# bdwsq1996/Effi-MVS-plus

Measured on NVIDIA B200. Metric: depth_maps_per_sec_1600x1184_5view, higher is better.
Workload: dtype hi+lo bf16 MMA x3, f32 accumulate (3-D regularization, fp32-grade) / f32 (warp, lookup, regression)

## Files before the change

### effi-mvs-plus_b200/capi.py

```python
from __future__ import annotations

import ctypes as C
import os

_HERE = os.path.dirname(os.path.abspath(__file__))
LIB_PATH = os.environ.get("EFFIMVS_LIB") or os.path.join(_HERE, "libeffimvs.so")

OK, EINVAL, EUNSUPPORTED, ECUDA, EWORKSPACE = 0, -1, -2, -3, -4
HYP_TENSOR, HYP_PLANES, HYP_LOCAL = 0, 1, 2
RANGE_SCALAR, RANGE_PIXEL = 0, 1
FEA_NCHW, FEA_NHWC = 0, 1
PREC_F32, PREC_BF16, PREC_BF16X3 = 0, 1, 2
WS_PREPARE, WS_RUN = 1, 2
CONV2D_BIAS, CONV2D_BIAS_RELU, CONV2D_ADD_RELU, CONV2D_GRU_GATES, CONV2D_GRU_UPDATE = 0, 1, 2, 3, 4
MAX_SRC_VIEWS = 16


class EffiMVSError(RuntimeError):
    def __init__(self, code, msg):
        super().__init__("libeffimvs error {}: {}".format(code, msg))
        self.code = code


if not os.path.exists(LIB_PATH):
    raise ImportError("libeffimvs.so is not built ({}); run __graft_entry__.build() -- the hot path has no "
                      "CPU or PyTorch fallback".format(LIB_PATH))

lib = C.CDLL(LIB_PATH)

_p, _i, _f, _sz = C.c_void_p, C.c_int, C.c_float, C.c_size_t
_pp = C.POINTER(C.c_void_p)

SIGNATURES = {
    "effimvs_last_error": (C.c_char_p, []),
    "effimvs_version": (_i, []),
    "effimvs_relative_projection_f32": (_i, [_p, _i, _i, _p, _p]),
    "effimvs_homo_warp_f32": (_i, [_p, _p, _p, _i, _i, _i, _i, _i, _i, _p, _p]),
    "effimvs_depth_range_samples_f32": (_i, [_p, _p, _i, _i, _i, _i, _p, _p]),
    "effimvs_depth_ranges_f32": (_i, [_p, _i, _i, _i, _p, _p, _p]),
    "effimvs_fusion_masks_f32": (_i, [_p, _p, _i, _i, _i, _i, _f, _f, _i, _i, _p, _p]),
    "effimvs_warp_corr_agg_f32": (_i, [_p, _pp, _i, _p, _p, _i, _p, _p, _i, _i, _i, _i, _i, _i, _i, _p, _p, _p]),
    "effimvs_warp_corr_views_f32": (_i, [_p, _pp, _i, _p, _p, _i, _i, _i, _i, _i, _i, _i, _p, _p, _p]),
    "effimvs_weighted_agg_f32": (_i, [_p, _p, _i, _i, _i, _i, _i, _p, _p]),
    "effimvs_volume_lookup_f32": (_i, [_p, _p, _p, _p, _i, _i, _i, _i, _i, _i, _i, _p, _p]),
    "effimvs_dynamic_cost_f32": (_i, [_p, _p, _p, _p, _p, _p, _i, _i, _i, _i, _i, _i, _p, _p]),
    "effimvs_softmax_regress_conf_f32": (_i, [_p, _p, _i, _i, _i, _i, _i, _p, _p, _p]),
    "effimvs_conv3d_f32": (_i, [_p, _p, _p, _p, _i, _i, _i, _i, _i, _i, _i, _i, _i, _i, _i, _p, _i, _i, _p]),
    "effimvs_conv3d_bf16_workspace_bytes": (_sz, [_i, _i, _i, _i, _i, _i, _i, _i, _i]),
    "effimvs_conv3d_bf16": (_i, [_p, _p, _p, _p, _i, _i, _i, _i, _i, _i, _i, _i, _i, _i, _p, _sz, _p, _p]),
    "effimvs_costreg_workspace_bytes": (_sz, [_i, _i, _i, _i, _i]),
    "effimvs_costreg_fpn3d": (_i, [_p, _pp, _pp, _i, _i, _i, _i, _i, _p, _sz, _p, _p]),
    "effimvs_cost_up_workspace_bytes": (_sz, [_i, _i, _i, _i, _i]),
    "effimvs_cost_up_small": (_i, [_p, _p, _pp, _pp, _i, _i, _i, _i, _i, _p, _sz, _p, _p]),
    "effimvs_costreg_fpn3d_ex": (_i, [_p, _pp, _pp, _i, _i, _i, _i, _i, _i, _p, _sz, _p, _p]),
    "effimvs_cost_up_small_ex": (_i, [_p, _p, _pp, _pp, _i, _i, _i, _i, _i, _i, _p, _sz, _p, _p]),
    "effimvs_gru_reset_f32": (_i, [_p, _p, _p, C.c_longlong, _i, _i, _p, _p]),
    "effimvs_gru_update_f32": (_i, [_p, _p, _p, _p, _p, C.c_longlong, _i, _i, _p, _p]),
    "effimvs_gru_delta_f32": (_i, [_p, _p, _p, _p, _p, _i, _i, _p, _p, _p]),
    "effimvs_inv_init_f32": (_i, [_p, _p, _p, _i, _i, _p, _p, _p]),
    "effimvs_delta_head_f32": (_i, [_p, _p, _p, _p, _p, _p, _i, _i, _i, _i, _p, _p, _p]),
    "effimvs_convex_upsample_f32": (_i, [_p, _p, _f, _p, _p, _p, _i, _i, _i, _i, _p, _p, _p]),
    "effimvs_convex_upsample_conv_f32": (_i, [_p, _i, _p, _p, _f, _p, _p, _p, _i, _i, _i, _i, _p, _p, _p]),
    "effimvs_encoder_head_f32": (_i, [_p, _p, _p, _p, _p, _p, _i, _i, _i, _i, _i, _p, _p]),
    "effimvs_encoder_head_hostw_f32": (_i, [_p, _p, _p, _i, _i, _i, _i, _i, _p, _p]),
    "effimvs_encoder_head_pack_host": (_i, [_p, _p, _p, _p, _i, _i, _p]),
    "effimvs_encoder_head_table_floats": (_i, [_i]),
    "effimvs_encoder_tail_f32": (_i, [_p, _p, _p, C.c_longlong, _i, _i, _p, _p]),
    "effimvs_encoder_tail_ctx_f32": (_i, [_p, _p, _p, _i, _i, _i, _p, _p, C.c_longlong, _i, _i, _p, _p]),
    "effimvs_conv2d_tf32_supported": (_i, [_i, _i]),
    "effimvs_conv2d_tf32_packed_bytes": (_sz, [_i, _i]),
    "effimvs_conv2d_tf32_pack": (_i, [_p, _i, _i, _p, _p]),
    "effimvs_conv2d_bf16x3_supported": (_i, [_i, _i]),
    "effimvs_conv2d_bf16x3_packed_bytes": (_sz, [_i, _i]),
    "effimvs_conv2d_bf16x3_pack": (_i, [_p, _i, _i, _p, _p]),
    "effimvs_conv2d_bf16x3": (_i, [_p, C.c_longlong, _i, _p, C.c_longlong, _i, _p, _p, _i, _i, _i, _i, _i,
                                   _p, C.c_longlong, _p, C.c_longlong, _p, C.c_longlong, _p]),
    "effimvs_conv2d_tf32": (_i, [_p, C.c_longlong, _i, _p, C.c_longlong, _i, _p, _p, _i, _i, _i, _i, _i,
                                 _p, C.c_longlong, _p, C.c_longlong, _p, C.c_longlong, _p]),
    "effimvs_gru_init_f32": (_i, [_p, C.c_longlong, _i, _i, _p, _p]),
    "effimvs_gru_init_ctx_f32": (_i, [_p, C.c_longlong, _i, _i, _p, _p, _p, _p, _p]),
    "effimvs_dtu_filter_f32": (_i, [_p, _p, _p, _p, C.POINTER(C.c_double), C.POINTER(C.c_float), _i, _i, _i, _f, _f, _i, _i, _i,
                                    _p, _p, _p, _p, _p, _p, _p]),
    "effimvs_images_u8_to_f32": (_i, [_p, C.c_longlong, _p, _p]),
    "effimvs_fusion_invert_cameras_f32": (_i, [_p, _p, _i, _i, _p, _p]),
    "effimvs_fusion_reproject_f32": (_i, [_p, _p, _p, _p, _p, _i, _i, _i, _i, _p, _p]),
    "effimvs_fusion_filter_f32": (_i, [_p, _p, _p, _p, _p, _p, _i, _i, _i, _i, _i, _i, _f, _f, _i, _f, _i, _p, _p, _p, _p, _p]),
}

for _name, (_res, _args) in SIGNATURES.items():
    _fn = getattr(lib, _name)
    _fn.restype = _res
    _fn.argtypes = _args


def last_error() -> str:
    return lib.effimvs_last_error().decode("utf-8", "replace")


def check(rc: int) -> None:
    if rc != OK:
        raise EffiMVSError(rc, last_error())


def ptr_array(ptrs):
    arr = (C.c_void_p * len(ptrs))(*[C.c_void_p(p) for p in ptrs])
    return C.cast(arr, _pp), arr
```

### effi-mvs-plus_b200/hotpath.py

```python
from __future__ import annotations

import collections
import functools
import os
import weakref

import torch

from . import capi, ops


def fold_bn(block, transposed: bool):
    bn = block.bn
    scale = bn.weight / torch.sqrt(bn.running_var + bn.eps)
    shift = bn.bias - bn.running_mean * scale
    w = block.conv.weight
    w = w * (scale.reshape(1, -1, 1, 1, 1) if transposed else scale.reshape(-1, 1, 1, 1, 1))
    return w.detach().float().contiguous(), shift.detach().float().contiguous()


class _FoldCache:

    def __init__(self):
        self._store = weakref.WeakKeyDictionary()

    def get(self, net, build):
        stamp = tuple((id(t), t._version, t.device) for t in list(net.parameters()) + list(net.buffers()))
        hit = self._store.get(net)
        if hit is None or hit[0] != stamp:
            hit = (stamp, build(net))
            self._store[net] = hit
        return hit[1]


def _inference_only(*tensors):
    if torch.is_grad_enabled() and any(torch.is_tensor(t) and t.requires_grad for t in tensors):
        raise RuntimeError("the CUDA hot path is inference only (no autograd formula): run it under torch.no_grad(), "
                           "or use upstream's PyTorch path for training / test-time adaptation")


class _WorkspaceCache:

    def __init__(self, cap: int = 24):
        self._store = collections.OrderedDict()
        self.cap = cap

    def get(self, key, nbytes, device):
        capturing = torch.cuda.is_current_stream_capturing() if torch.device(device).type == "cuda" else False
        ent = self._store.get(key)
        if ent is not None and ent["ws"].numel() < nbytes:
            if ent["pinned"]:
                raise RuntimeError("a regularization workspace captured in a CUDA graph is too small for this call")
            ent = None
        if ent is None:
            if capturing:
                raise RuntimeError("regularization workspace requested for the first time during CUDA-graph capture: "
                                   "run one eager forward of this shape before capturing")
            ent = {"ws": torch.empty(max(nbytes, 256), device=device, dtype=torch.uint8), "stamp": None, "pinned": False}
            self._store[key] = ent
            evictable = [k for k, e in self._store.items() if not e["pinned"] and k != key]
            while len(self._store) > self.cap and evictable:
                del self._store[evictable.pop(0)]
        ent["pinned"] = ent["pinned"] or capturing
        self._store.move_to_end(key)
        return ent

    def drop(self, owner_id):
        for k in [k for k in self._store if k[1] == owner_id]:
            del self._store[k]


def _is_planes(hyp: torch.Tensor) -> bool:
    return hyp.dim() == 2 or (hyp.dim() == 4 and (hyp.shape[2:] == (1, 1) or (hyp.stride(2) == 0 and hyp.stride(3) == 0)))


def _forget(hp_ref, owner_id):
    hp = hp_ref()
    if hp is not None:
        hp._tracked.discard(owner_id)
        hp._workspaces.drop(owner_id)


class CudaHotPath:
    name = "cuda"
    fused_update = True

    def __init__(self, precision: str = "f32", native_projection: bool = False, persistent_workspaces: bool = True,
                 parallel_branches: bool = False, conv2d_precision=None):
        self.precision = {"f32": capi.PREC_F32, "bf16": capi.PREC_BF16, "bf16x3": capi.PREC_BF16X3}[precision]
        self.native_projection = native_projection
        self.persistent_workspaces = persistent_workspaces and os.environ.get("EFFIMVS_PERSISTENT_WS", "1") != "0"
        self.parallel_branches = parallel_branches or os.environ.get("EFFIMVS_PARALLEL_BRANCHES", "0") == "1"
        self._folds = _FoldCache()
        self._workspaces = _WorkspaceCache()
        self._side_streams = {}
        self._tracked = set()
        if conv2d_precision not in (None, "bf16x3"):
            raise ValueError("conv2d_precision must be None or 'bf16x3', got {!r}".format(conv2d_precision))
        if conv2d_precision == "bf16x3":
            self.conv2d_precision = "bf16x3"
            self.conv2d_fp32_grade = True
            self.conv2d_tc = functools.partial(ops.conv2d_tc, precision="bf16x3")
            self.conv2d_tc_pack = functools.partial(ops.conv2d_tc_pack, precision="bf16x3")
            self.conv2d_tc_supported = functools.partial(ops.conv2d_tc_supported, precision="bf16x3")

    def side_stream(self, device):
        if not self.parallel_branches:
            return None
        key = torch.device(device).index
        if key not in self._side_streams:
            self._side_streams[key] = torch.cuda.Stream(device=device)
        return self._side_streams[key]

    def relative_projection(self, cams: torch.Tensor) -> torch.Tensor:
        if self.native_projection:
            return ops.relative_projection(cams)
        B, V = cams.shape[:2]

        def compose(c):
            P = c[:, 0].clone()
            P[:, :3, :4] = torch.matmul(c[:, 1, :3, :3], c[:, 0, :3, :4])
            return P
        inv_ref = torch.linalg.inv_ex(compose(cams[:, 0]))[0]
        rows = []
        for v in range(1, V):
            rel = torch.matmul(compose(cams[:, v]), inv_ref)
            rows.append(torch.cat([rel[:, :3, :3].reshape(B, 9), rel[:, :3, 3]], dim=-1))
        return torch.stack(rows, dim=1).contiguous()

    def stage1(self, features, cams, depth_hyp, pixel_wise_net, reg_net, G):
        if G != 1:
            raise ValueError("stage-1 view weighting requires G == 1 (upstream squeezes the group axis, Effi_MVS_plus.py:43)")
        _inference_only(*features)
        ref, srcs = features[0], list(features[1:])
        B, _, H, W = ref.shape
        D = depth_hyp.shape[1]
        proj = self.relative_projection(cams)
        if _is_planes(depth_hyp):
            hyp, mode = depth_hyp.reshape(B, D, -1)[:, :, 0].contiguous(), capi.HYP_PLANES
        else:
            hyp, mode = depth_hyp, capi.HYP_TENSOR
        sims, ent = ops.warp_corr_views(ref, srcs, proj, hyp, mode, D)
        n = len(srcs)
        vw = pixel_wise_net(ent.reshape(B * n, 1, H, W)).reshape(B, n, H, W)
        sim = ops.weighted_agg(sims, vw)
        prob_pre = self.cost_regularization(reg_net, sim.unsqueeze(1)).squeeze(1)
        depth, conf = ops.softmax_regress_conf(prob_pre, hyp, mode)
        return {"depth": depth, "photometric_confidence": conf, "view_weights": vw,
                "reg_volume": prob_pre, "volume": sim.unsqueeze(1)}

    def local_volume(self, cur_depth, features, cams, interval, view_weights, ndepth, G):
        _inference_only(cur_depth, *features)
        ref, srcs = features[0], list(features[1:])
        B, _, H, W = ref.shape
        proj = self.relative_projection(cams)
        iv = interval.reshape(-1).expand(B) if torch.is_tensor(interval) else torch.full((B,), float(interval), device=ref.device)
        sim, hyp = ops.warp_corr_agg(ref, srcs, proj, cur_depth, capi.HYP_LOCAL, iv.float().contiguous(), view_weights, ndepth, G, True)
        return sim.reshape(B, G * ndepth, H, W), hyp

    def warp_corr_agg(self, features, cams, hyp, view_weights, G):
        ref, srcs = features[0], list(features[1:])
        D = hyp.shape[1]
        proj = self.relative_projection(cams)
        if _is_planes(hyp):
            hyp, mode = hyp.reshape(hyp.shape[0], D, -1)[:, :, 0].contiguous(), capi.HYP_PLANES
        else:
            mode = capi.HYP_TENSOR
        return ops.warp_corr_agg(ref, srcs, proj, hyp, mode, None, view_weights, D, G, False)[0]

    def volume_lookup(self, volume, depth_sample, depth_min, depth_max):
        B, D, H, W = volume.shape
        base = getattr(depth_sample, "_base", None)
        if (not depth_sample.is_contiguous() and base is not None and base.is_contiguous() and base.dim() == 4
                and tuple(base.shape) == (B, depth_sample.shape[1], 2 * H, 2 * W)
                and depth_sample.stride() == (base.stride(0), base.stride(1), 2 * base.stride(2), 2)
                and depth_sample.storage_offset() == base.storage_offset()):
            return ops.volume_lookup(volume, base, self._range(depth_min, B), self._range(depth_max, B), 2)
        return ops.volume_lookup(volume, depth_sample, self._range(depth_min, B), self._range(depth_max, B), 1)

    @staticmethod
    def _range(t, B):
        t = t.reshape(B, -1)
        return t.contiguous()

    def dynamic_cost(self, cur_depth, raw_volume, reg_volume, interval, vmin, vmax, ndepth):
        B = raw_volume.shape[0]
        iv = interval.reshape(-1).expand(B) if torch.is_tensor(interval) else torch.full((B,), float(interval), device=raw_volume.device)
        return ops.dynamic_cost(cur_depth, raw_volume, reg_volume, iv.float().contiguous(), self._range(vmin, B), self._range(vmax, B), ndepth)

    def _reg_weights(self, net):
        def build(n):
            ws, bs = [], []
            for name, tr in (("conv0", False), ("conv1", False), ("conv2", False), ("conv3", False), ("conv4", False),
                             ("conv5", False), ("conv6", True), ("conv7", True)):
                w, b = fold_bn(getattr(n, name), tr)
                ws.append(w)
                bs.append(b)
            ws.append(n.prob.weight.detach().float().contiguous())
            return ws, bs
        return self._folds.get(net, build)

    def _csp_weights(self, net):
        def build(n):
            pairs = [fold_bn(n.conv0, False), fold_bn(n.conv_cost, False), fold_bn(n.conv1, False), fold_bn(n.conv2, True)]
            return [p[0] for p in pairs], [p[1] for p in pairs]
        return self._folds.get(net, build)

    def _track(self, net):
        if id(net) not in self._tracked:
            self._tracked.add(id(net))
            weakref.finalize(net, _forget, weakref.ref(self), id(net))

    def cost_regularization(self, net, x):
        ws, bs = self._reg_weights(net)
        if self.precision == capi.PREC_F32 or not self.persistent_workspaces:
            return ops.costreg_fpn3d(x, ws, bs, self.precision)
        B, _, D, H, W = x.shape
        self._track(net)
        ent = self._workspaces.get(("costreg", id(net), B, D, H, W, self.precision, x.device),
                                   ops.costreg_workspace_bytes(B, D, H, W, self.precision), x.device)
        if ent["stamp"] is not ws:
            ops.costreg_prepare(ws, bs, B, D, H, W, self.precision, ent["ws"])
            ent["stamp"] = ws
        return ops.costreg_run(x, ws, bs, self.precision, ent["ws"])

    def cross_scale(self, net, cur_volume, prev_resampled):
        ws, bs = self._csp_weights(net)
        if self.precision == capi.PREC_F32 or not self.persistent_workspaces:
            return ops.cost_up_small(cur_volume, prev_resampled, ws, bs, self.precision)
        B, _, D, H, W = cur_volume.shape
        self._track(net)
        ent = self._workspaces.get(("cost_up", id(net), B, D, H, W, self.precision, cur_volume.device),
                                   ops.cost_up_workspace_bytes(B, D, H, W, self.precision), cur_volume.device)
        if ent["stamp"] is not ws:
            ops.cost_up_prepare(ws, bs, B, D, H, W, self.precision, ent["ws"])
            ent["stamp"] = ws
        return ops.cost_up_run(cur_volume, prev_resampled, ws, bs, self.precision, ent["ws"])

    gru_reset = staticmethod(ops.gru_reset)
    gru_update = staticmethod(ops.gru_update)
    gru_delta = staticmethod(ops.gru_delta)
    inv_init = staticmethod(ops.inv_init)
    depth_ranges = staticmethod(ops.depth_ranges)
    delta_head = staticmethod(ops.delta_head)
    convex_upsample = staticmethod(ops.convex_upsample)
    convex_upsample_conv = staticmethod(ops.convex_upsample_conv)
    encoder_head = staticmethod(ops.encoder_head)
    encoder_tail = staticmethod(ops.encoder_tail)
    encoder_tail_ctx = staticmethod(ops.encoder_tail_ctx)
    gru_init = staticmethod(ops.gru_init)
    gru_init_ctx = staticmethod(ops.gru_init_ctx)
    conv2d_precision = "f16"
    conv2d_fp32_grade = False
    conv2d_tc = staticmethod(ops.conv2d_tc)
    conv2d_tc_pack = staticmethod(ops.conv2d_tc_pack)
    conv2d_tc_supported = staticmethod(ops.conv2d_tc_supported)

    def softmax_regress_conf(self, prob_pre, hyp):
        if _is_planes(hyp):
            B, D = prob_pre.shape[:2]
            return ops.softmax_regress_conf(prob_pre, hyp.reshape(B, D, -1)[:, :, 0].contiguous(), capi.HYP_PLANES)
        return ops.softmax_regress_conf(prob_pre, hyp, capi.HYP_TENSOR)
```

### effi-mvs-plus_b200/net.py

```python
from __future__ import annotations

import os

import torch
import torch.nn as nn
import torch.nn.functional as F

_FUSED_CONV_RELU = os.environ.get("EFFIMVS_FUSED_CONV_RELU", "1") == "1"


def conv_relu(x, weight, bias, stride=(1, 1), padding=(0, 0)):
    if _FUSED_CONV_RELU and x.is_cuda and bias is not None and not torch.is_grad_enabled():
        return torch.cudnn_convolution_relu(x, weight, bias, stride, padding, (1, 1), 1)
    return F.relu(F.conv2d(x, weight, bias, stride, padding), inplace=True)


def _conv_relu_mod(conv: nn.Conv2d, x):
    return conv_relu(x, conv.weight, conv.bias, conv.stride, conv.padding)


class ConvBNReLU2d(nn.Module):

    def __init__(self, cin, cout, k, stride=1, padding=0):
        super().__init__()
        self.conv = nn.Conv2d(cin, cout, k, stride=stride, padding=padding, bias=False)
        self.bn = nn.BatchNorm2d(cout)
        self._fold = None

    def _folded(self):
        bn = self.bn
        ts = (self.conv.weight, bn.weight, bn.bias, bn.running_mean, bn.running_var)
        stamp = tuple((id(t), t._version, t.device) for t in ts)
        if self._fold is None or self._fold[0] != stamp:
            scale = bn.weight / torch.sqrt(bn.running_var + bn.eps)
            w = (self.conv.weight * scale.reshape(-1, 1, 1, 1)).detach()
            b = (bn.bias - bn.running_mean * scale).detach()
            if w.is_cuda:
                w = w.contiguous(memory_format=torch.channels_last)
            self._fold = (stamp, w, b)
        return self._fold[1], self._fold[2]

    def forward(self, x):
        if self.training or torch.is_grad_enabled():
            return F.relu(self.bn(self.conv(x)), inplace=True)
        w, b = self._folded()
        return conv_relu(x, w, b, self.conv.stride, self.conv.padding)


class ConvBN3d(nn.Module):

    def __init__(self, cin, cout, transposed=False):
        super().__init__()
        if transposed:
            self.conv = nn.ConvTranspose3d(cin, cout, 3, bias=False)
        else:
            self.conv = nn.Conv3d(cin, cout, 3, bias=False)
        self.bn = nn.BatchNorm3d(cout)
        self.transposed = transposed


class RegNet3D(nn.Module):

    def __init__(self, cin=1, base=8):
        super().__init__()
        self.conv0 = ConvBN3d(cin, base)
        self.conv1 = ConvBN3d(base, base)
        self.conv2 = ConvBN3d(base, base * 2)
        self.conv3 = ConvBN3d(base * 2, base * 2)
        self.conv4 = ConvBN3d(base * 2, base * 4)
        self.conv5 = ConvBN3d(base * 4, base * 4)
        self.conv6 = ConvBN3d(base * 4, base * 2, transposed=True)
        self.conv7 = ConvBN3d(base * 2, base, transposed=True)
        self.prob = nn.Conv3d(base, 1, 3, stride=1, padding=1, bias=False)


class CrossScaleNet3D(nn.Module):

    def __init__(self, cin=1, base=8):
        super().__init__()
        self.conv0 = ConvBN3d(cin, base)
        self.conv_cost = ConvBN3d(1, base)
        self.conv1 = ConvBN3d(base * 2, base)
        self.conv2 = ConvBN3d(base, 1, transposed=True)


def _upsample2_nearest(t):
    N, C, h, w = t.shape
    v = t.permute(0, 2, 3, 1)
    v = v[:, :, None, :, None, :].expand(N, h, 2, w, 2, C).reshape(N, 2 * h, 2 * w, C)
    return v.permute(0, 3, 1, 2)


class FeaturePyramid(nn.Module):

    def __init__(self, chans, heads):
        super().__init__()
        c0, c1, c2, c3 = chans
        self.conv0 = nn.Sequential(ConvBNReLU2d(3, c0, 3, 1, 1), ConvBNReLU2d(c0, c0, 3, 1, 1))
        self.conv1 = nn.Sequential(ConvBNReLU2d(c0, c1, 5, 2, 2), ConvBNReLU2d(c1, c1, 3, 1, 1), ConvBNReLU2d(c1, c1, 3, 1, 1))
        self.conv2 = nn.Sequential(ConvBNReLU2d(c1, c2, 5, 2, 2), ConvBNReLU2d(c2, c2, 3, 1, 1), ConvBNReLU2d(c2, c2, 3, 1, 1))
        self.conv3 = nn.Sequential(ConvBNReLU2d(c2, c3, 5, 2, 2), ConvBNReLU2d(c3, c3, 3, 1, 1), ConvBNReLU2d(c3, c3, 3, 1, 1))
        self.out1 = nn.Conv2d(c3, heads[0], 1, bias=False)
        self.inner1 = nn.Conv2d(c2, c3, 1, bias=True)
        self.inner2 = nn.Conv2d(c1, c3, 1, bias=True)
        self.out2 = nn.Conv2d(c3, heads[1], 3, padding=1, bias=False)
        self.out3 = nn.Conv2d(c3, heads[2], 3, padding=1, bias=False)
        self.fused_topdown = None
        self._heads = None
        self._bias_maps = {}

    def _head_weights(self):
        ts = (self.out3.weight, self.inner2.weight, self.inner2.bias, self.inner1.weight, self.inner1.bias)
        stamp = tuple((id(t), t._version, t.device) for t in ts)
        if self._heads is None or self._heads[0] != stamp:
            w3 = self.out3.weight.detach()
            O, M = w3.shape[:2]
            lateral = torch.einsum("omyx,mi->oiyx", w3, self.inner2.weight.detach()[:, :, 0, 0]).contiguous()
            taps = {0: ((0, 0), (1, 1), (2, 1)), 1: ((0, 1), (1, 1), (2, 2))}
            phase = w3.new_zeros(2, 2, O, M, 3, 3)
            for py in (0, 1):
                for px in (0, 1):
                    for ky, dy in taps[py]:
                        for kx, dx in taps[px]:
                            phase[py, px, :, :, dy, dx] += w3[:, :, ky, kx]
            phase = phase.reshape(4 * O, M, 3, 3)
            w1t = self.inner1.weight.detach()[:, :, 0, 0].t().contiguous()
            if w3.is_cuda:
                lateral = lateral.contiguous(memory_format=torch.channels_last)
                phase = phase.contiguous(memory_format=torch.channels_last)
            self._heads = (stamp, lateral, phase, w1t)
            self._bias_maps = {}
        return self._heads[1:]

    def _bias_map(self, H, W):
        key = (H, W)
        if key not in self._bias_maps:
            b = self.inner2.bias.detach().reshape(1, -1, 1, 1).expand(1, -1, H, W)
            self._bias_maps[key] = F.conv2d(b, self.out3.weight.detach(), padding=1)
        return self._bias_maps[key]

    def _topdown_fused(self, l1, l2, top):
        lateral, phase, w1t = self._head_weights()
        s1 = self.out1(top)
        t2 = _upsample2_nearest(top + self.inner1.bias.reshape(1, -1, 1, 1))
        N, M, h, w = t2.shape
        t2_rows = t2.permute(0, 2, 3, 1).reshape(-1, M)
        t2_rows.addmm_(l2.permute(0, 2, 3, 1).reshape(-1, l2.shape[1]), w1t)
        s2 = self.out2(t2)
        O = self.out3.weight.shape[0]
        a = F.conv2d(t2, phase, padding=1)
        s3 = F.conv2d(l1, lateral, padding=1)
        s3_view = s3.permute(0, 2, 3, 1).reshape(N, h, 2, w, 2, O)
        if s3_view.data_ptr() != s3.data_ptr():
            return None
        s3_view += a.permute(0, 2, 3, 1).reshape(N, h, w, 2, 2, O).permute(0, 1, 3, 2, 4, 5)
        s3 += self._bias_map(2 * h, 2 * w)
        return [s1, s2, s3]

    def forward(self, x):
        l1 = self.conv1(self.conv0(x))
        l2 = self.conv2(l1)
        top = self.conv3(l2)
        fused = self.fused_topdown
        if fused is None:
            fused = x.is_cuda and not self.training and not torch.is_grad_enabled()
        if fused and l1.shape[2] == 2 * l2.shape[2] and l1.shape[3] == 2 * l2.shape[3]:
            out = self._topdown_fused(l1, l2, top)
            if out is not None:
                return out
        s1 = self.out1(top)
        top = F.interpolate(top, scale_factor=2, mode="nearest") + self.inner1(l2)
        s2 = self.out2(top)
        top = F.interpolate(top, scale_factor=2, mode="nearest") + self.inner2(l1)
        s3 = self.out3(top)
        return [s1, s2, s3]


class CostEncoder(nn.Module):

    def __init__(self, cost_dim, hidden, context_dim):
        super().__init__()
        self.convc1 = nn.Conv2d(cost_dim, hidden, 1)
        self.convc2 = nn.Conv2d(hidden, hidden, 3, padding=1)
        self.convd1 = nn.Conv2d(1, hidden, 7, padding=3)
        self.convd2 = nn.Conv2d(hidden, hidden, 3, padding=1)
        self.convd = nn.Conv2d(2 * hidden, hidden - context_dim, 3, padding=1)
        self.convc = nn.Conv2d(hidden, hidden, 1)

    def forward(self, inv_depth, cost, context):
        c = _conv_relu_mod(self.convc2, _conv_relu_mod(self.convc1, cost))
        d = _conv_relu_mod(self.convd2, _conv_relu_mod(self.convd1, inv_depth))
        m = self.convd(torch.cat([c, d], dim=1))
        return _conv_relu_mod(self.convc, torch.cat([m, context], dim=1))


class GRUCell2d(nn.Module):

    def __init__(self, hidden, inp):
        super().__init__()
        self.convz = nn.Conv2d(hidden + inp, hidden, 3, padding=1)
        self.convr = nn.Conv2d(hidden + inp, hidden, 3, padding=1)
        self.convq = nn.Conv2d(hidden + inp, hidden, 3, padding=1)

    def forward(self, h, x):
        hx = torch.cat([h, x], dim=1)
        z = torch.sigmoid(self.convz(hx))
        r = torch.sigmoid(self.convr(hx))
        q = torch.tanh(self.convq(torch.cat([r * h, x], dim=1)))
        return (1 - z) * h + z * q


class DeltaHead(nn.Module):

    def __init__(self, hidden):
        super().__init__()
        self.conv1 = nn.Conv2d(hidden, hidden, 3, padding=1)
        self.conv2 = nn.Conv2d(hidden, 1, 3, padding=1)

    def forward(self, x):
        return torch.tanh(self.conv2(_conv_relu_mod(self.conv1, x)))


class UpdateBlock(nn.Module):

    def __init__(self, hidden, cost_dim, ratio, context_dim):
        super().__init__()
        self.encoder = CostEncoder(cost_dim, hidden, context_dim)
        self.depth_gru = GRUCell2d(hidden, hidden)
        self.depth_head = DeltaHead(hidden)
        self.mask = nn.Sequential(nn.Conv2d(hidden, hidden * 2, 3, padding=1), nn.ReLU(inplace=True),
                                  nn.Conv2d(hidden * 2, ratio * ratio * 9, 1))

    def forward(self, net, cost_fn, inv_depth, context, iters, to_depth):
        inv_seq = []
        for _ in range(iters):
            inv_depth = inv_depth.detach()
            x = self.encoder(inv_depth, cost_fn(to_depth(inv_depth)), context)
            net = self.depth_gru(net, x)
            inv_depth = inv_depth + self.depth_head(net)
            inv_seq.append(inv_depth)
        return net, 0.25 * self.mask[2](_conv_relu_mod(self.mask[0], net)), inv_seq

    def forward_fused(self, glue, net, cost_fn, inv_depth, context, iters, lo_disp, hi_disp, ctx_map=None, want_mask=True, cur_depth=None):
        return update_block_forward_fused(self, glue, net, cost_fn, inv_depth, context, iters, lo_disp, hi_disp, ctx_map, want_mask, cur_depth)


def _fused_update_weights(block):
    g, e = block.depth_gru, block.encoder
    ts = (g.convz.weight, g.convz.bias, g.convr.weight, g.convr.bias, e.convd.bias, e.convc.weight, e.convc.bias,
          e.convc2.weight, e.convc2.bias, e.convd2.weight, e.convd2.bias, block.depth_head.conv2.weight,
          e.convd.weight, g.convq.weight, block.depth_head.conv1.weight, block.mask[0].weight)
    stamp = tuple((id(t), t._version, t.device) for t in ts)
    hit = getattr(block, "_effimvs_fused", None)
    if hit is None or hit[0] != stamp:
        cl = lambda w: w.detach().contiguous(memory_format=torch.channels_last)
        h = g.convz.out_channels
        hm = e.convd.out_channels
        wc = e.convc.weight.detach()
        bias_c = e.convc.bias.detach() + wc[:, :hm, 0, 0] @ e.convd.bias.detach()
        w_cd2 = wc.new_zeros(2 * h, 2 * h, 3, 3)
        w_cd2[:h, :h] = e.convc2.weight.detach()
        w_cd2[h:, h:] = e.convd2.weight.detach()
        hit = (stamp, {
            "w_cd2": cl(w_cd2), "b_cd2": torch.cat([e.convc2.bias.detach(), e.convd2.bias.detach()]).contiguous(),
            "wzr": cl(torch.cat([g.convz.weight, g.convr.weight], dim=0)),
            "wc_m": cl(wc[:, :hm]), "wc_ctx": cl(wc[:, hm:]), "bias_c": bias_c.contiguous(),
            "w_d2": block.depth_head.conv2.weight.detach().contiguous()})
        object.__setattr__(block, "_effimvs_fused", hit)
    return hit[1]


def _conv_tc_enabled(glue, h, H, W):
    env = os.environ.get("EFFIMVS_CONV2D", "auto")
    if env == "0" or not hasattr(glue, "conv2d_tc") or h % 16 != 0:
        return False
    if env != "1" and not torch.backends.cudnn.allow_tf32 and not getattr(glue, "conv2d_fp32_grade", False):
        return False
    sup = glue.conv2d_tc_supported
    if not (sup(2 * h, 2 * h) and sup(2 * h, h) and sup(h, h) and sup(h, 2 * h)):
        return False
    return env == "1" or H * W >= int(os.environ.get("EFFIMVS_CONV2D_MIN_PIXELS", "100000"))


def _tc_update_weights(block, glue, w):
    key = ("tc", getattr(glue, "conv2d_precision", "f16"))
    tc = w.get(key)
    if tc is None:
        g, e, hd = block.depth_gru, block.encoder, block.depth_head
        hm = e.convd.out_channels
        d_prime = torch.einsum("om,miyx->oiyx", e.convc.weight.detach()[:, :hm, 0, 0], e.convd.weight.detach())
        tc = {"cd2": glue.conv2d_tc_pack(w["w_cd2"]), "dprime": glue.conv2d_tc_pack(d_prime.contiguous()),
              "zr": glue.conv2d_tc_pack(w["wzr"]), "q": glue.conv2d_tc_pack(g.convq.weight.detach()),
              "head1": glue.conv2d_tc_pack(hd.conv1.weight.detach()), "mask0": glue.conv2d_tc_pack(block.mask[0].weight.detach()),
              "b_zr": torch.cat([g.convz.bias.detach(), g.convr.bias.detach()]).contiguous()}
        w[key] = tc
    return tc


def _start_inverse_depth(glue, inv_depth, cur_depth, lo_disp, hi_disp):
    if cur_depth is not None and hasattr(glue, "inv_init") and os.environ.get("EFFIMVS_INV_INIT", "1") != "0":
        return glue.inv_init(cur_depth, lo_disp, hi_disp)
    if inv_depth is None:
        lo, hi = lo_disp.reshape(-1, 1, 1, 1), hi_disp.reshape(-1, 1, 1, 1)
        inv_depth = (cur_depth.reciprocal() - lo) / ((hi - lo) + 1e-10)
    return glue.gru_delta(None, None, inv_depth, lo_disp, hi_disp)


def _update_block_forward_tc(block, glue, w, hx, ctx_term, cost_fn, inv_depth, iters, lo_disp, hi_disp, want_mask, cur_depth=None):
    from . import capi
    g, e, hd = block.depth_gru, block.encoder, block.depth_head
    tc = _tc_update_weights(block, glue, w)
    B, two_h, H, W = hx.shape
    h = two_h // 2
    ratio = int(round((block.mask[2].out_channels / 9) ** 0.5))
    mk = lambda c: torch.empty(B, c, H, W, device=hx.device, dtype=torch.float32, memory_format=torch.channels_last)
    cd, z, rh, t1 = mk(two_h), mk(h), mk(h), mk(h)
    net_v, x_v = hx[:, :h], hx[:, h:]
    cd2_cudnn = os.environ.get("EFFIMVS_CONV2D_CD2", "own") == "cudnn"
    inv, depth = _start_inverse_depth(glue, inv_depth, cur_depth, lo_disp, hi_disp)
    inv_seq, depth_seq = [], []
    for it in range(iters):
        c1d1 = glue.encoder_head(cost_fn(depth, it), inv, e.convc1.weight, e.convc1.bias, e.convd1.weight, e.convd1.bias)
        if cd2_cudnn:
            cd = conv_relu(c1d1, w["w_cd2"], w["b_cd2"], (1, 1), (1, 1))
        else:
            glue.conv2d_tc(c1d1, None, tc["cd2"], w["b_cd2"], two_h, capi.CONV2D_BIAS_RELU, cd, None, None)
        glue.conv2d_tc(cd, None, tc["dprime"], None, h, capi.CONV2D_ADD_RELU, x_v, ctx_term, None)
        glue.conv2d_tc(hx, None, tc["zr"], tc["b_zr"], two_h, capi.CONV2D_GRU_GATES, rh, net_v, z)
        glue.conv2d_tc(rh, x_v, tc["q"], g.convq.bias, h, capi.CONV2D_GRU_UPDATE, net_v, z, None)
        glue.conv2d_tc(net_v, None, tc["head1"], hd.conv1.bias, h, capi.CONV2D_BIAS_RELU, t1, None, None)
        inv, depth = glue.delta_head(t1, w["w_d2"], hd.conv2.bias, inv, lo_disp, hi_disp)
        inv_seq.append(inv)
        depth_seq.append(depth)
    m0 = mk(two_h)
    glue.conv2d_tc(net_v, None, tc["mask0"], block.mask[0].bias, two_h, capi.CONV2D_BIAS_RELU, m0, None, None)
    mask_pre = F.conv2d(m0, block.mask[2].weight, None)
    up, depth_up = glue.convex_upsample(mask_pre, block.mask[2].bias, 0.25, inv, lo_disp, hi_disp, ratio)
    return net_v, inv_seq, depth_seq, up, depth_up, (mask_pre if want_mask else None)


def update_block_forward_fused(block, glue, net, cost_fn, inv_depth, context, iters, lo_disp, hi_disp, ctx_map=None, want_mask=True,
                               cur_depth=None):
    w = _fused_update_weights(block)
    g, e, hd = block.depth_gru, block.encoder, block.depth_head
    ratio = int(round((block.mask[2].out_channels / 9) ** 0.5))
    h = g.convz.out_channels
    cx = e.convc.in_channels - e.convd.out_channels
    tail_ctx = hasattr(glue, "encoder_tail_ctx") and cx in (4, 8, 12) and os.environ.get("EFFIMVS_TAIL_CTX", "1") != "0"
    fused_start = ctx_map is not None and tail_ctx and hasattr(glue, "gru_init") and ctx_map.shape[1] == h + cx and h % 4 == 0
    Hm, Wm = (ctx_map if ctx_map is not None else net).shape[2:]
    tc_path = _conv_tc_enabled(glue, h, Hm, Wm) and tuple(hd.conv2.weight.shape) == (1, h, 3, 3) and h <= 128
    if fused_start and tc_path and hasattr(glue, "gru_init_ctx") and os.environ.get("EFFIMVS_INIT_CTX", "1") != "0":
        hx, ctx_term = glue.gru_init_ctx(ctx_map, h, w["wc_ctx"], w["bias_c"])
        return _update_block_forward_tc(block, glue, w, hx, ctx_term, cost_fn, inv_depth, iters, lo_disp, hi_disp, want_mask, cur_depth)
    if fused_start:
        hx = glue.gru_init(ctx_map, h)
        net = hx[:, :h]
        ctx_src, ctx_off, ctx_relu = ctx_map, h, True
    else:
        if ctx_map is not None:
            hidden, context = torch.split(ctx_map, [h, ctx_map.shape[1] - h], dim=1)
            net, context = torch.tanh(hidden), torch.relu(context)
        B, _, H, W = net.shape
        hx = torch.empty(B, 2 * h, H, W, device=net.device, dtype=net.dtype, memory_format=torch.channels_last)
        hx[:, :h] = net
        ctx_src = context.contiguous(memory_format=torch.channels_last) if (tail_ctx and context.is_cuda) else context
        ctx_off, ctx_relu = 0, False
    if tc_path:
        ctx_in = torch.relu(ctx_src[:, ctx_off:ctx_off + cx]) if ctx_relu else (ctx_src if ctx_src.shape[1] == cx else ctx_src[:, ctx_off:ctx_off + cx])
        ctx_term = F.conv2d(ctx_in, w["wc_ctx"], w["bias_c"]).contiguous(memory_format=torch.channels_last)
        return _update_block_forward_tc(block, glue, w, hx, ctx_term, cost_fn, inv_depth, iters, lo_disp, hi_disp, want_mask, cur_depth)
    if not tail_ctx:
        ctx_term = F.conv2d(context, w["wc_ctx"], w["bias_c"])
    inv, depth = _start_inverse_depth(glue, inv_depth, cur_depth, lo_disp, hi_disp)
    inv_seq, depth_seq = [], []
    head_fused = (hasattr(glue, "delta_head") and h % 16 == 0 and h <= 128 and tuple(hd.conv2.weight.shape) == (1, h, 3, 3)
                  and os.environ.get("EFFIMVS_DELTA_HEAD", "1") != "0")
    for it in range(iters):
        c1d1 = glue.encoder_head(cost_fn(depth, it), inv, e.convc1.weight, e.convc1.bias, e.convd1.weight, e.convd1.bias)
        cd = conv_relu(c1d1, w["w_cd2"], w["b_cd2"], (1, 1), (1, 1))
        m = F.conv2d(cd, e.convd.weight, None, padding=1)
        if tail_ctx:
            glue.encoder_tail_ctx(m, w["wc_m"], ctx_src, ctx_off, cx, ctx_relu, w["wc_ctx"], w["bias_c"], hx)
        else:
            glue.encoder_tail(m, w["wc_m"], ctx_term, hx)
        zr_pre = F.conv2d(hx, w["wzr"], None, padding=1)
        rhx = glue.gru_reset(zr_pre, g.convr.bias, hx)
        q_pre = F.conv2d(rhx, g.convq.weight, None, padding=1)
        net = glue.gru_update(zr_pre, g.convz.bias, q_pre, g.convq.bias, hx)
        if head_fused:
            inv, depth = glue.delta_head(_conv_relu_mod(hd.conv1, net), w["w_d2"], hd.conv2.bias, inv, lo_disp, hi_disp)
        else:
            pre = F.conv2d(_conv_relu_mod(hd.conv1, net), hd.conv2.weight, None, padding=1)
            inv, depth = glue.gru_delta(pre, hd.conv2.bias, inv, lo_disp, hi_disp)
        inv_seq.append(inv)
        depth_seq.append(depth)
    m0 = _conv_relu_mod(block.mask[0], net)
    if (not want_mask and hasattr(glue, "convex_upsample_conv") and tuple(block.mask[2].kernel_size) == (1, 1) and m0.shape[1] % 4 == 0
            and os.environ.get("EFFIMVS_UPSAMPLE_CONV", "0") == "1"):
        up, depth_up = glue.convex_upsample_conv(m0, block.mask[2].weight, block.mask[2].bias, 0.25, inv, lo_disp, hi_disp, ratio)
        return net, inv_seq, depth_seq, up, depth_up, None
    mask_pre = F.conv2d(m0, block.mask[2].weight, None)
    up, depth_up = glue.convex_upsample(mask_pre, block.mask[2].bias, 0.25, inv, lo_disp, hi_disp, ratio)
    return net, inv_seq, depth_seq, up, depth_up, mask_pre


def convex_upsample(x, mask, ratio):
    N, _, H, W = x.shape
    m = torch.softmax(mask.view(N, 1, 9, ratio, ratio, H, W), dim=2)
    nb = F.unfold(x, [3, 3], padding=1).view(N, 1, 9, 1, 1, H, W)
    up = torch.sum(m * nb, dim=2).permute(0, 1, 4, 2, 5, 3)
    return up.reshape(N, ratio * H, ratio * W)


class EffiMVSPlus(nn.Module):

    RATIOS = (4, 2, 1)
    HIDDEN = (48, 32, 16)
    CONTEXT = (12, 8, 4)
    FEAT = (32, 16, 8)
    G = 1

    def __init__(self, args, hotpath=None):
        super().__init__()
        self.ndepths = [int(e) for e in str(args.ndepths).split(",")]
        self.iters = [int(e) for e in str(args.GRUiters).split(",")]
        self.cost_num = int(args.CostNum)
        self.PixelwiseNet = nn.Sequential(ConvBNReLU2d(1, 16, 3, 1, 1), ConvBNReLU2d(16, 16, 3, 1, 1),
                                          ConvBNReLU2d(16, 8, 3, 1, 1), nn.Conv2d(8, 1, 1), nn.Sigmoid())
        self.feature = FeaturePyramid((8, 16, 32, 64), self.FEAT)
        self.cnet_depth = FeaturePyramid((4, 8, 16, 32), (60, 40, 20))
        blocks = [UpdateBlock(self.HIDDEN[i], self.G * self.cost_num * 2, 2, self.CONTEXT[i]) for i in range(3)]
        self.update_block_depth1, self.update_block_depth2, self.update_block_depth3 = blocks
        self.update_block = nn.ModuleList(blocks)
        self.CSP_R1, self.CSP_R2 = CrossScaleNet3D(self.G), CrossScaleNet3D(self.G)
        self.CSP_R = nn.ModuleList([self.CSP_R1, self.CSP_R2])
        self.CSP_C1, self.CSP_C2 = CrossScaleNet3D(self.G), CrossScaleNet3D(self.G)
        self.CSP_C = nn.ModuleList([self.CSP_C1, self.CSP_C2])
        self.cost_regularization = RegNet3D(self.G, 8)
        object.__setattr__(self, "_hotpath", hotpath)

    @property
    def hotpath(self):
        hp = self._hotpath
        if hp is None:
            from .hotpath import CudaHotPath
            hp = CudaHotPath()
            object.__setattr__(self, "_hotpath", hp)
        return hp

    def set_hotpath(self, hp):
        object.__setattr__(self, "_hotpath", hp)

    def encode(self, imgs):
        B, V = imgs.shape[:2]
        x = imgs.reshape(B * V, *imgs.shape[2:])
        if x.is_cuda:
            x = x.contiguous(memory_format=torch.channels_last)
        pyr = self.feature(x)
        return [[p.reshape(B, V, *p.shape[1:])[:, v] for v in range(V)] for p in pyr]

    def forward(self, imgs, proj_matrices, depth_values):
        return self.forward_from_features(self.encode(imgs), imgs[:, 0], proj_matrices, depth_values)

    def forward_from_features(self, feats, ref_img, proj_matrices, depth_values):
        hp = self.hotpath
        imgs = ref_img
        B = imgs.shape[0]
        disp_min = depth_values[:, 0].reshape(B, 1, 1, 1)
        disp_max = depth_values[:, -1].reshape(B, 1, 1, 1)
        planes = None
        if (hasattr(hp, "depth_ranges") and depth_values.is_cuda and not torch.is_grad_enabled()
                and os.environ.get("EFFIMVS_DEPTH_RANGES", "1") != "0"):
            R = hp.depth_ranges(depth_values, self.ndepths[0], [float(r) for r in self.RATIOS])
            row = lambda i: R[i * B:(i + 1) * B].reshape(B, 1, 1, 1)
            depth_far, depth_near, lo_disp, hi_disp = row(0), row(1), row(2), row(3)
            intervals = [row(4), row(5), row(6)]
            planes = R[8 * B:].reshape(B, self.ndepths[0])
        else:
            depth_far, depth_near = disp_min.reciprocal(), disp_max.reciprocal()
            unit = (disp_max - disp_min) / depth_values.size(1)
            intervals = [unit * r for r in self.RATIOS]
            lo_disp, hi_disp = depth_far.reciprocal(), depth_near.reciprocal()

        def to_depth(inv):
            return 1.0 / (lo_disp + (hi_disp - lo_disp) * inv).clamp(min=1e-4)

        ctx_pyr = self.cnet_depth(ref_img.contiguous(memory_format=torch.channels_last) if ref_img.is_cuda else ref_img)

        preds = []
        conf = None
        view_w = raw_vol = reg_vol = None
        vol_near, vol_far = depth_near, depth_far
        for s in range(3):
            f = feats[s]
            cams = proj_matrices["stage{}".format(s + 1)]
            glue = hp if (getattr(hp, "fused_update", False) and imgs.is_cuda and not torch.is_grad_enabled()) else None
            if glue is None:
                hidden, context = torch.split(ctx_pyr[s], [self.HIDDEN[s], self.CONTEXT[s]], dim=1)
                hidden, context = torch.tanh(hidden), torch.relu(context)
            H, W = f[0].shape[2:]
            if s == 0:
                D = self.ndepths[0]
                if planes is None:
                    k = torch.arange(D, device=imgs.device, dtype=imgs.dtype).reshape(1, D)
                    inv_s = disp_min.reshape(B, 1) + k * ((disp_max - disp_min).reshape(B, 1) / (D - 1))
                    planes = inv_s.reciprocal()
                hyp = planes.reshape(B, D, 1, 1).expand(B, D, H, W)
                out = hp.stage1(f, cams, hyp, self.PixelwiseNet, self.cost_regularization, self.G)
                conf = F.interpolate(out["photometric_confidence"].unsqueeze(1), [H * 4, W * 4], mode="nearest").squeeze(1)
                view_w = out["view_weights"]
                raw_vol = out["volume"].squeeze(1)
                reg_vol = out["reg_volume"]
                cur_depth = out["depth"].unsqueeze(1)
                preds.append(out["depth"])
            else:
                cur_depth = preds[-1].unsqueeze(1).detach()
                view_w = F.interpolate(view_w, scale_factor=2, mode="nearest")
                D = self.ndepths[s]
                loc, hyp = hp.local_volume(cur_depth, f, cams, intervals[s], view_w, D, self.G)
                hyp_low = hyp[:, :, ::2, ::2]
                loc5 = loc.reshape(B, self.G, D, H, W)
                side = hp.side_stream(loc.device) if hasattr(hp, "side_stream") else None
                if side is not None:
                    main = torch.cuda.current_stream(loc.device)
                    side.wait_stream(main)
                    with torch.cuda.stream(side):
                        raw_prev = hp.volume_lookup(raw_vol, hyp_low, vol_near, vol_far)
                        raw_vol = hp.cross_scale(self.CSP_C[s - 1], loc5, raw_prev.unsqueeze(1)).squeeze(1)
                reg_prev = hp.volume_lookup(reg_vol, hyp_low, vol_near, vol_far)
                reg_vol = hp.cross_scale(self.CSP_R[s - 1], loc5, reg_prev.unsqueeze(1)).squeeze(1)
                if side is not None:
                    main.wait_stream(side)
                else:
                    raw_prev = hp.volume_lookup(raw_vol, hyp_low, vol_near, vol_far)
                    raw_vol = hp.cross_scale(self.CSP_C[s - 1], loc5, raw_prev.unsqueeze(1)).squeeze(1)
                vol_far, vol_near = hyp[:, 0:1], hyp[:, -1:]

            interval = intervals[s]

            def cost_fn(depth, _it=0, _raw=raw_vol, _reg=reg_vol, _iv=interval, _n=vol_near, _f=vol_far):
                return hp.dynamic_cost(depth, _raw, _reg, _iv, _n, _f, self.cost_num)

            if glue is not None:
                _, _, depth_seq, _, depth_up, _ = self.update_block[s].forward_fused(
                    glue, None, cost_fn, None, None, self.iters[s], lo_disp.reshape(B), hi_disp.reshape(B), ctx_pyr[s], False, cur_depth)
                preds.extend(d.squeeze(1) for d in depth_seq)
                preds.append(depth_up)
                continue
            inv0 = (cur_depth.reciprocal() - lo_disp) / ((hi_disp - lo_disp) + 1e-10)
            _, mask, inv_seq = self.update_block[s](hidden, cost_fn, inv0, context, self.iters[s], to_depth)
            for inv in inv_seq:
                preds.append(to_depth(inv).squeeze(1))
            up = convex_upsample(inv_seq[-1], mask, 2).unsqueeze(1)
            preds.append(to_depth(up).squeeze(1))
        return {"depth": preds, "photometric_confidence": conf}
```

### effi-mvs-plus_b200/ops.py

```python
from __future__ import annotations

import os
from typing import List, Optional, Tuple

import torch
from torch import Tensor

from . import capi

_lib = capi.lib
_NHWC_MAXC = int(os.environ.get("EFFIMVS_NHWC_MAXC", "32"))

LAUNCHES = 0


def _count(n: int) -> None:
    global LAUNCHES
    LAUNCHES += n


def _dev(t: Tensor, name: str) -> Tensor:
    if not t.is_cuda:
        raise RuntimeError("effimvs::{} got a CPU tensor; the hot path is CUDA-only (no fallback)".format(name))
    if t.dtype != torch.float32:
        t = t.float()
    return t.contiguous()


def _features(ref: Tensor, srcs: List[Tensor], name: str):
    for t in [ref] + list(srcs):
        if not t.is_cuda:
            raise RuntimeError("effimvs::{} got a CPU tensor; the hot path is CUDA-only (no fallback)".format(name))
    nhwc = (ref.dim() == 4 and 1 < ref.shape[1] <= _NHWC_MAXC and not ref.is_contiguous()
            and ref.is_contiguous(memory_format=torch.channels_last))
    fmt = torch.channels_last if nhwc else torch.contiguous_format
    fix = lambda t: (t if t.dtype == torch.float32 else t.float()).contiguous(memory_format=fmt)
    return fix(ref), [fix(s) for s in srcs], (capi.FEA_NHWC if nhwc else capi.FEA_NCHW)


def _stream() -> int:
    return torch.cuda.current_stream().cuda_stream


def _on_tensor_device(fn):
    import functools

    def tensors(args):
        for a in args:
            if isinstance(a, Tensor):
                yield a
            elif isinstance(a, (list, tuple)):
                for b in a:
                    if isinstance(b, Tensor):
                        yield b

    @functools.wraps(fn)
    def call(*args, **kw):
        devs = {t.device for t in tensors(list(args) + list(kw.values())) if t.is_cuda}
        if len(devs) > 1:
            raise RuntimeError("effimvs::{} got tensors on several devices: {}".format(fn.__name__, sorted(map(str, devs))))
        if not devs or next(iter(devs)).index == torch.cuda.current_device():
            return fn(*args, **kw)
        with torch.cuda.device(next(iter(devs))):
            return fn(*args, **kw)
    return call


def _opt(t: Optional[Tensor]):
    return t.data_ptr() if t is not None else None


@torch.library.custom_op("effimvs::relative_projection", mutates_args=())
@_on_tensor_device
def relative_projection(cams: Tensor) -> Tensor:
    cams = _dev(cams, "relative_projection")
    B, V = cams.shape[0], cams.shape[1]
    out = torch.empty(B, V - 1, 12, device=cams.device, dtype=torch.float32)
    _count(1)
    capi.check(_lib.effimvs_relative_projection_f32(cams.data_ptr(), B, V, out.data_ptr(), _stream()))
    return out


@relative_projection.register_fake
def _(cams):
    return cams.new_empty(cams.shape[0], cams.shape[1] - 1, 12)


@torch.library.custom_op("effimvs::homo_warp", mutates_args=())
@_on_tensor_device
def homo_warp(src_fea: Tensor, proj: Tensor, hyp: Tensor, hyp_mode: int, D: int) -> Tensor:
    src_fea, proj, hyp = _dev(src_fea, "homo_warp"), _dev(proj, "homo_warp"), _dev(hyp, "homo_warp")
    B, Cc, H, W = src_fea.shape
    out = torch.empty(B, Cc, D, H, W, device=src_fea.device, dtype=torch.float32)
    _count(1)
    capi.check(_lib.effimvs_homo_warp_f32(src_fea.data_ptr(), proj.data_ptr(), hyp.data_ptr(), hyp_mode, B, Cc, H, W, D,
                                          out.data_ptr(), _stream()))
    return out


@homo_warp.register_fake
def _(src_fea, proj, hyp, hyp_mode, D):
    B, Cc, H, W = src_fea.shape
    return src_fea.new_empty(B, Cc, D, H, W)


@torch.library.custom_op("effimvs::depth_ranges", mutates_args=())
@_on_tensor_device
def depth_ranges(depth_values: Tensor, ndepth1: int, ratios: List[float]) -> Tensor:
    import ctypes
    depth_values = _dev(depth_values, "depth_ranges")
    B, Dv = depth_values.shape
    if len(ratios) != 3:
        raise ValueError("depth_ranges: three interval ratios expected")
    out = torch.empty(B * (8 + ndepth1), device=depth_values.device, dtype=torch.float32)
    r3 = (ctypes.c_float * 3)(*[float(r) for r in ratios])
    _count(1)
    capi.check(_lib.effimvs_depth_ranges_f32(depth_values.data_ptr(), B, Dv, ndepth1, r3, out.data_ptr(), _stream()))
    return out


@depth_ranges.register_fake
def _(depth_values, ndepth1, ratios):
    return depth_values.new_empty(depth_values.shape[0] * (8 + ndepth1))


@torch.library.custom_op("effimvs::depth_range_samples", mutates_args=())
@_on_tensor_device
def depth_range_samples(cur: Tensor, interval: Tensor, ndepth: int) -> Tensor:
    cur, interval = _dev(cur, "depth_range_samples"), _dev(interval, "depth_range_samples")
    B, H, W = cur.shape
    out = torch.empty(B, ndepth, H, W, device=cur.device, dtype=torch.float32)
    _count(1)
    capi.check(_lib.effimvs_depth_range_samples_f32(cur.data_ptr(), interval.data_ptr(), B, ndepth, H, W, out.data_ptr(), _stream()))
    return out


@depth_range_samples.register_fake
def _(cur, interval, ndepth):
    B, H, W = cur.shape
    return cur.new_empty(B, ndepth, H, W)


@torch.library.custom_op("effimvs::fusion_masks", mutates_args=())
@_on_tensor_device
def fusion_masks(ref_depth: Tensor, reproj_xyd: Tensor, dist_base: float, rel_diff_base: float, thres_view: int,
                 relative: bool) -> Tensor:
    ref_depth, reproj_xyd = _dev(ref_depth, "fusion_masks"), _dev(reproj_xyd, "fusion_masks")
    n, v, _, h, w = reproj_xyd.shape
    K = v - thres_view + 1
    out = torch.empty(n, v, K, h, w, device=ref_depth.device, dtype=torch.uint8)
    _count(1)
    capi.check(_lib.effimvs_fusion_masks_f32(ref_depth.data_ptr(), reproj_xyd.data_ptr(), n, v, h, w, dist_base, rel_diff_base,
                                             thres_view, int(relative), out.data_ptr(), _stream()))
    return out


@fusion_masks.register_fake
def _(ref_depth, reproj_xyd, dist_base, rel_diff_base, thres_view, relative):
    n, v, _, h, w = reproj_xyd.shape
    return ref_depth.new_empty(n, v, v - thres_view + 1, h, w, dtype=torch.uint8)


@torch.library.custom_op("effimvs::warp_corr_agg", mutates_args=())
@_on_tensor_device
def warp_corr_agg(ref: Tensor, srcs: List[Tensor], proj: Tensor, hyp: Tensor, hyp_mode: int,
                  interval: Optional[Tensor], weights: Optional[Tensor], D: int, G: int,
                  want_hyp: bool) -> Tuple[Tensor, Tensor]:
    ref, srcs, layout = _features(ref, srcs, "warp_corr_agg")
    proj, hyp = _dev(proj, "warp_corr_agg"), _dev(hyp, "warp_corr_agg")
    interval = _dev(interval, "warp_corr_agg") if interval is not None else None
    weights = _dev(weights, "warp_corr_agg") if weights is not None else None
    B, Cc, H, W = ref.shape
    sim = torch.empty(B, G, D, H, W, device=ref.device, dtype=torch.float32)
    hyp_out = torch.empty(B, D, H, W, device=ref.device, dtype=torch.float32) if want_hyp else ref.new_empty(0)
    arr, keep = capi.ptr_array([s.data_ptr() for s in srcs])
    _count(1)
    capi.check(_lib.effimvs_warp_corr_agg_f32(ref.data_ptr(), arr, len(srcs), proj.data_ptr(), hyp.data_ptr(), hyp_mode,
                                              _opt(interval), _opt(weights), B, Cc, H, W, D, G, layout, sim.data_ptr(),
                                              hyp_out.data_ptr() if want_hyp else None, _stream()))
    del keep
    return sim, hyp_out


@warp_corr_agg.register_fake
def _(ref, srcs, proj, hyp, hyp_mode, interval, weights, D, G, want_hyp):
    B, _, H, W = ref.shape
    return ref.new_empty(B, G, D, H, W), (ref.new_empty(B, D, H, W) if want_hyp else ref.new_empty(0))


@torch.library.custom_op("effimvs::warp_corr_views", mutates_args=())
@_on_tensor_device
def warp_corr_views(ref: Tensor, srcs: List[Tensor], proj: Tensor, hyp: Tensor, hyp_mode: int, D: int) -> Tuple[Tensor, Tensor]:
    ref, srcs, layout = _features(ref, srcs, "warp_corr_views")
    proj, hyp = _dev(proj, "warp_corr_views"), _dev(hyp, "warp_corr_views")
    B, Cc, H, W = ref.shape
    n = len(srcs)
    sims = torch.empty(B, n, D, H, W, device=ref.device, dtype=torch.float32)
    ent = torch.empty(B, n, H, W, device=ref.device, dtype=torch.float32)
    arr, keep = capi.ptr_array([s.data_ptr() for s in srcs])
    _count(1)
    capi.check(_lib.effimvs_warp_corr_views_f32(ref.data_ptr(), arr, n, proj.data_ptr(), hyp.data_ptr(), hyp_mode,
                                                B, Cc, H, W, D, layout, sims.data_ptr(), ent.data_ptr(), _stream()))
    del keep
    return sims, ent


@warp_corr_views.register_fake
def _(ref, srcs, proj, hyp, hyp_mode, D):
    B, _, H, W = ref.shape
    return ref.new_empty(B, len(srcs), D, H, W), ref.new_empty(B, len(srcs), H, W)


@torch.library.custom_op("effimvs::weighted_agg", mutates_args=())
@_on_tensor_device
def weighted_agg(sims: Tensor, weights: Tensor) -> Tensor:
    sims, weights = _dev(sims, "weighted_agg"), _dev(weights, "weighted_agg")
    B, n, D, H, W = sims.shape
    out = torch.empty(B, D, H, W, device=sims.device, dtype=torch.float32)
    _count(1)
    capi.check(_lib.effimvs_weighted_agg_f32(sims.data_ptr(), weights.data_ptr(), B, n, D, H, W, out.data_ptr(), _stream()))
    return out


@weighted_agg.register_fake
def _(sims, weights):
    B, n, D, H, W = sims.shape
    return sims.new_empty(B, D, H, W)


def _range_mode(dmin: Tensor, B: int, H: int, W: int) -> int:
    if dmin.numel() == B:
        return capi.RANGE_SCALAR
    if dmin.numel() == B * H * W:
        return capi.RANGE_PIXEL
    raise ValueError("depth range must have B or B*H*W elements, got {}".format(tuple(dmin.shape)))


@torch.library.custom_op("effimvs::volume_lookup", mutates_args=())
@_on_tensor_device
def volume_lookup(volume: Tensor, depth_sample: Tensor, depth_min: Tensor, depth_max: Tensor, sample_stride: int) -> Tensor:
    volume, depth_sample = _dev(volume, "volume_lookup"), _dev(depth_sample, "volume_lookup")
    depth_min, depth_max = _dev(depth_min, "volume_lookup"), _dev(depth_max, "volume_lookup")
    B, D, H, W = volume.shape
    d = depth_sample.shape[1]
    if tuple(depth_sample.shape[2:]) != (H * sample_stride, W * sample_stride):
        raise ValueError("depth_sample {} does not match volume {} with stride {}".format(tuple(depth_sample.shape), tuple(volume.shape), sample_stride))
    mode = _range_mode(depth_min, B, H, W)
    if _range_mode(depth_max, B, H, W) != mode:
        raise ValueError("depth_min and depth_max must have the same shape")
    out = torch.empty(B, d, H, W, device=volume.device, dtype=torch.float32)
    _count(1)
    capi.check(_lib.effimvs_volume_lookup_f32(volume.data_ptr(), depth_sample.data_ptr(), depth_min.data_ptr(),
                                              depth_max.data_ptr(), mode, sample_stride, B, D, d, H, W, out.data_ptr(), _stream()))
    return out


@volume_lookup.register_fake
def _(volume, depth_sample, depth_min, depth_max, sample_stride):
    B, D, H, W = volume.shape
    return volume.new_empty(B, depth_sample.shape[1], H, W)


@torch.library.custom_op("effimvs::dynamic_cost", mutates_args=())
@_on_tensor_device
def dynamic_cost(cur_depth: Tensor, raw: Tensor, reg: Tensor, interval: Tensor, depth_min: Tensor, depth_max: Tensor,
                 ndepth: int) -> Tensor:
    cur_depth, raw, reg = _dev(cur_depth, "dynamic_cost"), _dev(raw, "dynamic_cost"), _dev(reg, "dynamic_cost")
    interval, depth_min, depth_max = _dev(interval, "dynamic_cost"), _dev(depth_min, "dynamic_cost"), _dev(depth_max, "dynamic_cost")
    B, D, H, W = raw.shape
    if reg.shape != raw.shape or cur_depth.numel() != B * H * W or interval.numel() != B:
        raise ValueError("dynamic_cost: inconsistent shapes")
    mode = _range_mode(depth_min, B, H, W)
    if _range_mode(depth_max, B, H, W) != mode:
        raise ValueError("depth_min and depth_max must have the same shape")
    out = torch.empty(B, 2 * ndepth, H, W, device=raw.device, dtype=torch.float32)
    _count(1)
    capi.check(_lib.effimvs_dynamic_cost_f32(cur_depth.data_ptr(), raw.data_ptr(), reg.data_ptr(), interval.data_ptr(),
                                             depth_min.data_ptr(), depth_max.data_ptr(), mode, ndepth, B, D, H, W,
                                             out.data_ptr(), _stream()))
    return out


@dynamic_cost.register_fake
def _(cur_depth, raw, reg, interval, depth_min, depth_max, ndepth):
    B, D, H, W = raw.shape
    return raw.new_empty(B, 2 * ndepth, H, W)


@torch.library.custom_op("effimvs::softmax_regress_conf", mutates_args=())
@_on_tensor_device
def softmax_regress_conf(prob_pre: Tensor, hyp: Tensor, hyp_mode: int) -> Tuple[Tensor, Tensor]:
    prob_pre, hyp = _dev(prob_pre, "softmax_regress_conf"), _dev(hyp, "softmax_regress_conf")
    B, D, H, W = prob_pre.shape
    depth = torch.empty(B, H, W, device=prob_pre.device, dtype=torch.float32)
    conf = torch.empty(B, H, W, device=prob_pre.device, dtype=torch.float32)
    _count(1)
    capi.check(_lib.effimvs_softmax_regress_conf_f32(prob_pre.data_ptr(), hyp.data_ptr(), hyp_mode, B, D, H, W,
                                                     depth.data_ptr(), conf.data_ptr(), _stream()))
    return depth, conf


@softmax_regress_conf.register_fake
def _(prob_pre, hyp, hyp_mode):
    B, D, H, W = prob_pre.shape
    return prob_pre.new_empty(B, H, W), prob_pre.new_empty(B, H, W)


@torch.library.custom_op("effimvs::conv3d", mutates_args=())
@_on_tensor_device
def conv3d(x: Tensor, weight: Tensor, bias: Optional[Tensor], residual: Optional[Tensor], stride: List[int],
           transposed: bool, relu: bool) -> Tensor:
    x, weight = _dev(x, "conv3d"), _dev(weight, "conv3d")
    bias = _dev(bias, "conv3d") if bias is not None else None
    residual = _dev(residual, "conv3d") if residual is not None else None
    B, Cin, D, H, W = x.shape
    Cout = weight.shape[1] if transposed else weight.shape[0]
    sd, sh, sw = stride
    if transposed:
        Do, Ho, Wo = D * sd, H * sh, W * sw
    else:
        Do, Ho, Wo = (D - 1) // sd + 1, (H - 1) // sh + 1, (W - 1) // sw + 1
    y = torch.empty(B, Cout, Do, Ho, Wo, device=x.device, dtype=torch.float32)
    _count(1)
    capi.check(_lib.effimvs_conv3d_f32(x.data_ptr(), weight.data_ptr(), _opt(bias), _opt(residual), B, Cin, Cout, D, H, W,
                                       sd, sh, sw, int(transposed), int(relu), y.data_ptr(), 0, Cout, _stream()))
    return y


@conv3d.register_fake
def _(x, weight, bias, residual, stride, transposed, relu):
    B, Cin, D, H, W = x.shape
    Cout = weight.shape[1] if transposed else weight.shape[0]
    sd, sh, sw = stride
    if transposed:
        return x.new_empty(B, Cout, D * sd, H * sh, W * sw)
    return x.new_empty(B, Cout, (D - 1) // sd + 1, (H - 1) // sh + 1, (W - 1) // sw + 1)


@torch.library.custom_op("effimvs::conv3d_bf16", mutates_args=())
@_on_tensor_device
def conv3d_bf16(x: Tensor, weight: Tensor, bias: Optional[Tensor], residual: Optional[Tensor], sd: int,
                transposed: bool, relu: bool, precision: int) -> Tensor:
    x, weight = _dev(x, "conv3d_bf16"), _dev(weight, "conv3d_bf16")
    bias = _dev(bias, "conv3d_bf16") if bias is not None else None
    residual = _dev(residual, "conv3d_bf16") if residual is not None else None
    B, Cin, D, H, W = x.shape
    Cout = weight.shape[1] if transposed else weight.shape[0]
    if transposed:
        Do, Ho, Wo = D * sd, H * 2, W * 2
    else:
        Do, Ho, Wo = D // sd, H // sd, W // sd
    need = _lib.effimvs_conv3d_bf16_workspace_bytes(B, Cin, Cout, D, H, W, sd, int(transposed), precision)
    ws = torch.empty(max(need, 256), device=x.device, dtype=torch.uint8)
    y = torch.empty(B, Cout, Do, Ho, Wo, device=x.device, dtype=torch.float32)
    _count(5)
    capi.check(_lib.effimvs_conv3d_bf16(x.data_ptr(), weight.data_ptr(), _opt(bias), _opt(residual), B, Cin, Cout, D, H, W,
                                        sd, int(transposed), int(relu), precision, ws.data_ptr(), ws.numel(), y.data_ptr(), _stream()))
    return y


@conv3d_bf16.register_fake
def _(x, weight, bias, residual, sd, transposed, relu, precision):
    B, Cin, D, H, W = x.shape
    Cout = weight.shape[1] if transposed else weight.shape[0]
    if transposed:
        return x.new_empty(B, Cout, D * sd, H * 2, W * 2)
    return x.new_empty(B, Cout, D // sd, H // sd, W // sd)


@torch.library.custom_op("effimvs::costreg_fpn3d", mutates_args=())
@_on_tensor_device
def costreg_fpn3d(x: Tensor, weights: List[Tensor], biases: List[Tensor], precision: int) -> Tensor:
    x = _dev(x, "costreg_fpn3d")
    weights = [_dev(w, "costreg_fpn3d") for w in weights]
    biases = [_dev(b, "costreg_fpn3d") for b in biases]
    if len(weights) != 9 or len(biases) != 8:
        raise ValueError("costreg_fpn3d wants 9 weights and 8 biases")
    B, _, D, H, W = x.shape
    need = _lib.effimvs_costreg_workspace_bytes(B, D, H, W, precision)
    ws = torch.empty(max(need, 256), device=x.device, dtype=torch.uint8)
    out = torch.empty(B, 1, D, H, W, device=x.device, dtype=torch.float32)
    wa, k1 = capi.ptr_array([w.data_ptr() for w in weights])
    ba, k2 = capi.ptr_array([b.data_ptr() for b in biases])
    _count(9 if precision == capi.PREC_F32 else 11)
    capi.check(_lib.effimvs_costreg_fpn3d(x.data_ptr(), wa, ba, B, D, H, W, precision, ws.data_ptr(), ws.numel(),
                                          out.data_ptr(), _stream()))
    del k1, k2
    return out


@costreg_fpn3d.register_fake
def _(x, weights, biases, precision):
    return x.new_empty(x.shape)


@torch.library.custom_op("effimvs::cost_up_small", mutates_args=())
@_on_tensor_device
def cost_up_small(x: Tensor, prev: Tensor, weights: List[Tensor], biases: List[Tensor], precision: int) -> Tensor:
    x, prev = _dev(x, "cost_up_small"), _dev(prev, "cost_up_small")
    weights = [_dev(w, "cost_up_small") for w in weights]
    biases = [_dev(b, "cost_up_small") for b in biases]
    if len(weights) != 4 or len(biases) != 4:
        raise ValueError("cost_up_small wants 4 weights and 4 biases")
    B, _, D, H, W = x.shape
    if tuple(prev.shape) != (B, 1, D, H // 2, W // 2):
        raise ValueError("cost_up_small: prev {} does not match x {}".format(tuple(prev.shape), tuple(x.shape)))
    need = _lib.effimvs_cost_up_workspace_bytes(B, D, H, W, precision)
    ws = torch.empty(max(need, 256), device=x.device, dtype=torch.uint8)
    out = torch.empty(B, 1, D, H, W, device=x.device, dtype=torch.float32)
    wa, k1 = capi.ptr_array([w.data_ptr() for w in weights])
    ba, k2 = capi.ptr_array([b.data_ptr() for b in biases])
    _count(4 if precision == capi.PREC_F32 else 6)
    capi.check(_lib.effimvs_cost_up_small(x.data_ptr(), prev.data_ptr(), wa, ba, B, D, H, W, precision, ws.data_ptr(),
                                          ws.numel(), out.data_ptr(), _stream()))
    del k1, k2
    return out


@cost_up_small.register_fake
def _(x, prev, weights, biases, precision):
    return x.new_empty(x.shape)


def costreg_workspace_bytes(B: int, D: int, H: int, W: int, precision: int) -> int:
    return int(_lib.effimvs_costreg_workspace_bytes(B, D, H, W, precision))


def cost_up_workspace_bytes(B: int, D: int, H: int, W: int, precision: int) -> int:
    return int(_lib.effimvs_cost_up_workspace_bytes(B, D, H, W, precision))


def _wsbuf(ws: Tensor, what: str) -> Tensor:
    if not ws.is_cuda or ws.dtype != torch.uint8 or not ws.is_contiguous():
        raise RuntimeError("effimvs::{}: the workspace must be a contiguous CUDA uint8 tensor".format(what))
    return ws


def _reg_args(weights, biases, nw, nb, what):
    weights = [_dev(w, what) for w in weights]
    biases = [_dev(b, what) for b in biases]
    if len(weights) != nw or len(biases) != nb:
        raise ValueError("{} wants {} weights and {} biases".format(what, nw, nb))
    return capi.ptr_array([w.data_ptr() for w in weights]), capi.ptr_array([b.data_ptr() for b in biases])


@torch.library.custom_op("effimvs::costreg_prepare", mutates_args=("ws",))
@_on_tensor_device
def costreg_prepare(weights: List[Tensor], biases: List[Tensor], B: int, D: int, H: int, W: int, precision: int, ws: Tensor) -> None:
    (wa, k1), (ba, k2) = _reg_args(weights, biases, 9, 8, "costreg_prepare")
    ws = _wsbuf(ws, "costreg_prepare")
    _count(0 if precision == capi.PREC_F32 else 2)
    capi.check(_lib.effimvs_costreg_fpn3d_ex(None, wa, ba, B, D, H, W, precision, capi.WS_PREPARE, ws.data_ptr(), ws.numel(),
                                             None, _stream()))
    del k1, k2


@torch.library.custom_op("effimvs::costreg_run", mutates_args=("ws",))
@_on_tensor_device
def costreg_run(x: Tensor, weights: List[Tensor], biases: List[Tensor], precision: int, ws: Tensor) -> Tensor:
    x, ws = _dev(x, "costreg_run"), _wsbuf(ws, "costreg_run")
    (wa, k1), (ba, k2) = _reg_args(weights, biases, 9, 8, "costreg_run")
    B, _, D, H, W = x.shape
    out = torch.empty(B, 1, D, H, W, device=x.device, dtype=torch.float32)
    _count(9)
    capi.check(_lib.effimvs_costreg_fpn3d_ex(x.data_ptr(), wa, ba, B, D, H, W, precision, capi.WS_RUN, ws.data_ptr(), ws.numel(),
                                             out.data_ptr(), _stream()))
    del k1, k2
    return out


@costreg_run.register_fake
def _(x, weights, biases, precision, ws):
    return x.new_empty(x.shape)


@torch.library.custom_op("effimvs::cost_up_prepare", mutates_args=("ws",))
@_on_tensor_device
def cost_up_prepare(weights: List[Tensor], biases: List[Tensor], B: int, D: int, H: int, W: int, precision: int, ws: Tensor) -> None:
    (wa, k1), (ba, k2) = _reg_args(weights, biases, 4, 4, "cost_up_prepare")
    ws = _wsbuf(ws, "cost_up_prepare")
    _count(0 if precision == capi.PREC_F32 else 2)
    capi.check(_lib.effimvs_cost_up_small_ex(None, None, wa, ba, B, D, H, W, precision, capi.WS_PREPARE, ws.data_ptr(), ws.numel(),
                                             None, _stream()))
    del k1, k2


@torch.library.custom_op("effimvs::cost_up_run", mutates_args=("ws",))
@_on_tensor_device
def cost_up_run(x: Tensor, prev: Tensor, weights: List[Tensor], biases: List[Tensor], precision: int, ws: Tensor) -> Tensor:
    x, prev, ws = _dev(x, "cost_up_run"), _dev(prev, "cost_up_run"), _wsbuf(ws, "cost_up_run")
    (wa, k1), (ba, k2) = _reg_args(weights, biases, 4, 4, "cost_up_run")
    B, _, D, H, W = x.shape
    if tuple(prev.shape) != (B, 1, D, H // 2, W // 2):
        raise ValueError("cost_up_run: prev {} does not match x {}".format(tuple(prev.shape), tuple(x.shape)))
    out = torch.empty(B, 1, D, H, W, device=x.device, dtype=torch.float32)
    _count(4)
    capi.check(_lib.effimvs_cost_up_small_ex(x.data_ptr(), prev.data_ptr(), wa, ba, B, D, H, W, precision, capi.WS_RUN, ws.data_ptr(),
                                             ws.numel(), out.data_ptr(), _stream()))
    del k1, k2
    return out


@cost_up_run.register_fake
def _(x, prev, weights, biases, precision, ws):
    return x.new_empty(x.shape)


@torch.library.custom_op("effimvs::images_u8_to_f32", mutates_args=("out",))
@_on_tensor_device
def images_u8_to_f32(images: Tensor, out: Tensor) -> None:
    if not (images.is_cuda and out.is_cuda):
        raise RuntimeError("effimvs::images_u8_to_f32 got a CPU tensor; the hot path is CUDA-only (no fallback)")
    if images.dtype != torch.uint8 or out.dtype != torch.float32 or images.shape != out.shape or not (
            images.is_contiguous() and out.is_contiguous()):
        raise RuntimeError("effimvs::images_u8_to_f32: images must be uint8, out fp32, same shape, contiguous")
    _count(1)
    capi.check(_lib.effimvs_images_u8_to_f32(images.data_ptr(), images.numel(), out.data_ptr(), _stream()))


@torch.library.custom_op("effimvs::fusion_invert_cameras", mutates_args=())
@_on_tensor_device
def fusion_invert_cameras(ref_cam: Tensor, srcs_cam: Tensor) -> Tensor:
    ref_cam, srcs_cam = _dev(ref_cam, "fusion_invert_cameras"), _dev(srcs_cam, "fusion_invert_cameras")
    n, v = srcs_cam.shape[0], srcs_cam.shape[1]
    out = torch.empty(n, v + 1, 2, 4, 4, device=ref_cam.device, dtype=torch.float32)
    _count(1)
    capi.check(_lib.effimvs_fusion_invert_cameras_f32(ref_cam.data_ptr(), srcs_cam.data_ptr(), n, v, out.data_ptr(), _stream()))
    return out


@fusion_invert_cameras.register_fake
def _(ref_cam, srcs_cam):
    return ref_cam.new_empty(srcs_cam.shape[0], srcs_cam.shape[1] + 1, 2, 4, 4)


@torch.library.custom_op("effimvs::fusion_reproject", mutates_args=())
@_on_tensor_device
def fusion_reproject(ref_depth: Tensor, srcs_depth: Tensor, ref_cam: Tensor, srcs_cam: Tensor,
                     inv_cams: Optional[Tensor]) -> Tensor:
    ref_depth, srcs_depth = _dev(ref_depth, "fusion_reproject"), _dev(srcs_depth, "fusion_reproject")
    ref_cam, srcs_cam = _dev(ref_cam, "fusion_reproject"), _dev(srcs_cam, "fusion_reproject")
    inv_cams = _dev(inv_cams, "fusion_reproject") if inv_cams is not None else None
    n, v, _, h, w = srcs_depth.shape
    out = torch.empty(n, v, 3, h, w, device=ref_depth.device, dtype=torch.float32)
    _count(1)
    capi.check(_lib.effimvs_fusion_reproject_f32(ref_depth.data_ptr(), srcs_depth.data_ptr(), ref_cam.data_ptr(),
                                                 srcs_cam.data_ptr(), _opt(inv_cams), n, v, h, w, out.data_ptr(), _stream()))
    return out


@fusion_reproject.register_fake
def _(ref_depth, srcs_depth, ref_cam, srcs_cam, inv_cams):
    n, v, _, h, w = srcs_depth.shape
    return ref_depth.new_empty(n, v, 3, h, w)


@torch.library.custom_op("effimvs::fusion_filter", mutates_args=())
@_on_tensor_device
def fusion_filter(ref_depth: Tensor, srcs_depth: Tensor, conf: Tensor, ref_cam: Tensor, srcs_cam: Tensor,
                  inv_cams: Optional[Tensor], dist_base: float, rel_diff_base: float, thres_view: int,
                  prob_threshold: float, relative: bool, want_masks: bool) -> Tuple[Tensor, Tensor, Tensor, Tensor]:
    ref_depth, srcs_depth, conf = _dev(ref_depth, "fusion_filter"), _dev(srcs_depth, "fusion_filter"), _dev(conf, "fusion_filter")
    ref_cam, srcs_cam = _dev(ref_cam, "fusion_filter"), _dev(srcs_cam, "fusion_filter")
    inv_cams = _dev(inv_cams, "fusion_filter") if inv_cams is not None else None
    n, v, _, h, w = srcs_depth.shape
    hc, wc = conf.shape[-2:]
    dev = ref_depth.device
    final = torch.empty(n, 1, h, w, device=dev, dtype=torch.uint8)
    avg = torch.empty(n, 1, h, w, device=dev, dtype=torch.float32)
    pts = torch.empty(n, 3, h, w, device=dev, dtype=torch.float32)
    K = v - thres_view + 1
    masks = torch.empty((n, v, K, h, w) if want_masks else (0,), device=dev, dtype=torch.uint8)
    _count(1)
    capi.check(_lib.effimvs_fusion_filter_f32(ref_depth.data_ptr(), srcs_depth.data_ptr(), conf.data_ptr(), ref_cam.data_ptr(),
                                              srcs_cam.data_ptr(), _opt(inv_cams), n, v, h, w, hc, wc, dist_base, rel_diff_base,
                                              thres_view, prob_threshold, int(relative), final.data_ptr(), avg.data_ptr(),
                                              pts.data_ptr(), masks.data_ptr() if want_masks else None, _stream()))
    return final, avg, pts, masks


@fusion_filter.register_fake
def _(ref_depth, srcs_depth, conf, ref_cam, srcs_cam, inv_cams, dist_base, rel_diff_base, thres_view, prob_threshold,
      relative, want_masks):
    n, v, _, h, w = srcs_depth.shape
    K = v - thres_view + 1
    u8 = torch.uint8
    return (ref_depth.new_empty(n, 1, h, w, dtype=u8), ref_depth.new_empty(n, 1, h, w), ref_depth.new_empty(n, 3, h, w),
            ref_depth.new_empty((n, v, K, h, w) if want_masks else (0,), dtype=u8))


def _nhwc(t: Tensor, name: str) -> Tensor:
    if not t.is_cuda:
        raise RuntimeError("effimvs::{} got a CPU tensor; the hot path is CUDA-only (no fallback)".format(name))
    if t.dtype != torch.float32:
        t = t.float()
    return t.contiguous(memory_format=torch.channels_last)


@torch.library.custom_op("effimvs::gru_reset", mutates_args=())
@_on_tensor_device
def gru_reset(zr_pre: Tensor, bias_r: Tensor, hx: Tensor) -> Tensor:
    zr_pre, hx, bias_r = _nhwc(zr_pre, "gru_reset"), _nhwc(hx, "gru_reset"), _dev(bias_r, "gru_reset")
    B, two_h, H, W = zr_pre.shape
    h = two_h // 2
    out = torch.empty_like(hx, memory_format=torch.channels_last)
    _count(1)
    capi.check(_lib.effimvs_gru_reset_f32(zr_pre.data_ptr(), bias_r.data_ptr(), hx.data_ptr(), B * H * W, h, hx.shape[1] - h,
                                          out.data_ptr(), _stream()))
    return out


@gru_reset.register_fake
def _(zr_pre, bias_r, hx):
    return torch.empty_like(hx, memory_format=torch.channels_last)


@torch.library.custom_op("effimvs::gru_update", mutates_args=("hx",))
@_on_tensor_device
def gru_update(zr_pre: Tensor, bias_z: Tensor, q_pre: Tensor, bias_q: Tensor, hx: Tensor) -> Tensor:
    zr_pre, q_pre = _nhwc(zr_pre, "gru_update"), _nhwc(q_pre, "gru_update")
    bias_z, bias_q = _dev(bias_z, "gru_update"), _dev(bias_q, "gru_update")
    if not (hx.is_cuda and hx.dtype == torch.float32 and hx.is_contiguous(memory_format=torch.channels_last)):
        raise RuntimeError("effimvs::gru_update needs hx as a channels-last fp32 CUDA tensor (it is updated in place)")
    B, h, H, W = q_pre.shape
    net = torch.empty_like(q_pre, memory_format=torch.channels_last)
    _count(1)
    capi.check(_lib.effimvs_gru_update_f32(zr_pre.data_ptr(), bias_z.data_ptr(), q_pre.data_ptr(), bias_q.data_ptr(), hx.data_ptr(),
                                           B * H * W, h, hx.shape[1] - h, net.data_ptr(), _stream()))
    return net


@gru_update.register_fake
def _(zr_pre, bias_z, q_pre, bias_q, hx):
    return torch.empty_like(q_pre, memory_format=torch.channels_last)


@torch.library.custom_op("effimvs::gru_delta", mutates_args=())
@_on_tensor_device
def gru_delta(pre: Optional[Tensor], bias: Optional[Tensor], inv: Tensor, lo_disp: Tensor, hi_disp: Tensor) -> Tuple[Tensor, Tensor]:
    inv, lo_disp, hi_disp = _dev(inv, "gru_delta"), _dev(lo_disp, "gru_delta"), _dev(hi_disp, "gru_delta")
    B, _, H, W = inv.shape
    if pre is not None:
        pre, bias = _dev(pre, "gru_delta"), _dev(bias, "gru_delta")
        inv_out = torch.empty_like(inv)
    else:
        inv_out = inv
    depth = torch.empty_like(inv)
    _count(1)
    capi.check(_lib.effimvs_gru_delta_f32(_opt(pre), _opt(bias), inv.data_ptr(), lo_disp.data_ptr(), hi_disp.data_ptr(), B, H * W,
                                          inv_out.data_ptr() if pre is not None else None, depth.data_ptr(), _stream()))
    return (inv_out if pre is not None else inv.clone()), depth


@gru_delta.register_fake
def _(pre, bias, inv, lo_disp, hi_disp):
    return torch.empty_like(inv), torch.empty_like(inv)


@torch.library.custom_op("effimvs::inv_init", mutates_args=())
@_on_tensor_device
def inv_init(cur_depth: Tensor, lo_disp: Tensor, hi_disp: Tensor) -> Tuple[Tensor, Tensor]:
    cur_depth, lo_disp, hi_disp = _dev(cur_depth, "inv_init"), _dev(lo_disp, "inv_init"), _dev(hi_disp, "inv_init")
    B, _, H, W = cur_depth.shape
    inv, depth = torch.empty_like(cur_depth), torch.empty_like(cur_depth)
    _count(1)
    capi.check(_lib.effimvs_inv_init_f32(cur_depth.data_ptr(), lo_disp.data_ptr(), hi_disp.data_ptr(), B, H * W, inv.data_ptr(),
                                         depth.data_ptr(), _stream()))
    return inv, depth


@inv_init.register_fake
def _(cur_depth, lo_disp, hi_disp):
    return torch.empty_like(cur_depth), torch.empty_like(cur_depth)


@torch.library.custom_op("effimvs::delta_head", mutates_args=())
@_on_tensor_device
def delta_head(t: Tensor, weight: Tensor, bias: Tensor, inv: Tensor, lo_disp: Tensor, hi_disp: Tensor) -> Tuple[Tensor, Tensor]:
    t, weight, bias = _nhwc(t, "delta_head"), _dev(weight, "delta_head"), _dev(bias, "delta_head")
    inv, lo_disp, hi_disp = _dev(inv, "delta_head"), _dev(lo_disp, "delta_head"), _dev(hi_disp, "delta_head")
    B, h, H, W = t.shape
    if tuple(weight.shape) != (1, h, 3, 3) or inv.numel() != B * H * W:
        raise ValueError("delta_head: weight {} / inv {} do not match t {}".format(tuple(weight.shape), tuple(inv.shape), tuple(t.shape)))
    inv_out, depth = torch.empty_like(inv), torch.empty_like(inv)
    _count(1)
    capi.check(_lib.effimvs_delta_head_f32(t.data_ptr(), weight.data_ptr(), bias.data_ptr(), inv.data_ptr(), lo_disp.data_ptr(),
                                           hi_disp.data_ptr(), B, h, H, W, inv_out.data_ptr(), depth.data_ptr(), _stream()))
    return inv_out, depth


@delta_head.register_fake
def _(t, weight, bias, inv, lo_disp, hi_disp):
    return torch.empty_like(inv), torch.empty_like(inv)


@torch.library.custom_op("effimvs::convex_upsample", mutates_args=())
@_on_tensor_device
def convex_upsample(mask_pre: Tensor, mask_bias: Optional[Tensor], mask_scale: float, inv: Tensor, lo_disp: Tensor,
                    hi_disp: Tensor, ratio: int) -> Tuple[Tensor, Tensor]:
    mask_pre, inv = _nhwc(mask_pre, "convex_upsample"), _dev(inv, "convex_upsample")
    lo_disp, hi_disp = _dev(lo_disp, "convex_upsample"), _dev(hi_disp, "convex_upsample")
    mask_bias = _dev(mask_bias, "convex_upsample") if mask_bias is not None else None
    B, _, H, W = inv.shape
    up = torch.empty(B, ratio * H, ratio * W, device=inv.device, dtype=torch.float32)
    depth = torch.empty_like(up)
    _count(1)
    capi.check(_lib.effimvs_convex_upsample_f32(mask_pre.data_ptr(), _opt(mask_bias), mask_scale, inv.data_ptr(), lo_disp.data_ptr(),
                                                hi_disp.data_ptr(), B, H, W, ratio, up.data_ptr(), depth.data_ptr(), _stream()))
    return up, depth


@convex_upsample.register_fake
def _(mask_pre, mask_bias, mask_scale, inv, lo_disp, hi_disp, ratio):
    B, _, H, W = inv.shape
    return inv.new_empty(B, ratio * H, ratio * W), inv.new_empty(B, ratio * H, ratio * W)


@torch.library.custom_op("effimvs::convex_upsample_conv", mutates_args=())
@_on_tensor_device
def convex_upsample_conv(t: Tensor, mask_w: Tensor, mask_bias: Optional[Tensor], mask_scale: float, inv: Tensor, lo_disp: Tensor,
                         hi_disp: Tensor, ratio: int) -> Tuple[Tensor, Tensor]:
    t, mask_w, inv = _nhwc(t, "convex_upsample_conv"), _dev(mask_w, "convex_upsample_conv"), _dev(inv, "convex_upsample_conv")
    lo_disp, hi_disp = _dev(lo_disp, "convex_upsample_conv"), _dev(hi_disp, "convex_upsample_conv")
    mask_bias = _dev(mask_bias, "convex_upsample_conv") if mask_bias is not None else None
    B, K, H, W = t.shape
    if mask_w.numel() != 9 * ratio * ratio * K or inv.numel() != B * H * W:
        raise ValueError("convex_upsample_conv: shapes do not match")
    up = torch.empty(B, ratio * H, ratio * W, device=inv.device, dtype=torch.float32)
    depth = torch.empty_like(up)
    _count(1)
    capi.check(_lib.effimvs_convex_upsample_conv_f32(t.data_ptr(), K, mask_w.data_ptr(), _opt(mask_bias), mask_scale, inv.data_ptr(),
                                                     lo_disp.data_ptr(), hi_disp.data_ptr(), B, H, W, ratio, up.data_ptr(),
                                                     depth.data_ptr(), _stream()))
    return up, depth


@convex_upsample_conv.register_fake
def _(t, mask_w, mask_bias, mask_scale, inv, lo_disp, hi_disp, ratio):
    B, _, H, W = inv.shape
    return inv.new_empty(B, ratio * H, ratio * W), inv.new_empty(B, ratio * H, ratio * W)


_EH_TABLES: dict = {}


def _encoder_head_table(ws, CD: int, h: int):
    import weakref
    key = tuple(id(t) for t in ws)
    stamp = tuple((t.data_ptr(), t._version) for t in ws)
    hit = _EH_TABLES.get(key)
    if hit is not None and hit[1] == stamp and all(r() is t for r, t in zip(hit[0], ws)):
        return hit[2]
    if torch.cuda.is_current_stream_capturing():
        return None
    host = [t.detach().to("cpu", torch.float32).contiguous() for t in ws]
    table = torch.empty(_lib.effimvs_encoder_head_table_floats(h), dtype=torch.float32)
    capi.check(_lib.effimvs_encoder_head_pack_host(host[0].data_ptr(), host[1].data_ptr(), host[2].data_ptr(), host[3].data_ptr(), CD, h,
                                                   table.data_ptr()))
    if len(_EH_TABLES) >= 256:
        for k in [k for k, v in _EH_TABLES.items() if any(r() is None for r in v[0])]:
            del _EH_TABLES[k]
    try:
        _EH_TABLES[key] = (tuple(weakref.ref(t) for t in ws), stamp, table)
    except TypeError:
        pass
    return table


@torch.library.custom_op("effimvs::encoder_head", mutates_args=())
@_on_tensor_device
def encoder_head(cost: Tensor, inv: Tensor, wc1: Tensor, bc1: Tensor, wd1: Tensor, bd1: Tensor) -> Tensor:
    cost, inv = _dev(cost, "encoder_head"), _dev(inv, "encoder_head")
    wc1, bc1, wd1, bd1 = _dev(wc1, "encoder_head"), _dev(bc1, "encoder_head"), _dev(wd1, "encoder_head"), _dev(bd1, "encoder_head")
    B, CD, H, W = cost.shape
    h = wc1.shape[0]
    out = torch.empty(B, 2 * h, H, W, device=cost.device, dtype=torch.float32, memory_format=torch.channels_last)
    mode = os.environ.get("EFFIMVS_EH_CONST", "auto")
    use_const = 1 <= CD <= 8 and h % 16 == 0 and 16 <= h <= 128 and (mode == "1" or (mode != "0" and h == 16))
    table = _encoder_head_table((wc1, bc1, wd1, bd1), CD, h) if use_const else None
    if table is not None:
        _count(h // 16)
        capi.check(_lib.effimvs_encoder_head_hostw_f32(cost.data_ptr(), inv.data_ptr(), table.data_ptr(), B, CD, h, H, W, out.data_ptr(),
                                                       _stream()))
        return out
    _count(1)
    capi.check(_lib.effimvs_encoder_head_f32(cost.data_ptr(), inv.data_ptr(), wc1.data_ptr(), bc1.data_ptr(), wd1.data_ptr(), bd1.data_ptr(),
                                             B, CD, h, H, W, out.data_ptr(), _stream()))
    return out


@encoder_head.register_fake
def _(cost, inv, wc1, bc1, wd1, bd1):
    B, _, H, W = cost.shape
    return torch.empty((B, 2 * wc1.shape[0], H, W), device=cost.device, dtype=cost.dtype, memory_format=torch.channels_last)


@torch.library.custom_op("effimvs::encoder_tail", mutates_args=("hx",))
@_on_tensor_device
def encoder_tail(m: Tensor, w: Tensor, ctx_term: Tensor, hx: Tensor) -> None:
    m, ctx_term, w = _nhwc(m, "encoder_tail"), _nhwc(ctx_term, "encoder_tail"), _dev(w, "encoder_tail")
    if not (hx.is_cuda and hx.dtype == torch.float32 and hx.is_contiguous(memory_format=torch.channels_last)):
        raise RuntimeError("effimvs::encoder_tail needs hx as a channels-last fp32 CUDA tensor (it is updated in place)")
    B, hm, H, W = m.shape
    h = ctx_term.shape[1]
    if hx.shape[1] != 2 * h or w.shape[0] != h or w.shape[1] != hm:
        raise ValueError("encoder_tail: shapes do not match")
    _count(1)
    capi.check(_lib.effimvs_encoder_tail_f32(m.data_ptr(), w.data_ptr(), ctx_term.data_ptr(), B * H * W, hm, h, hx.data_ptr(), _stream()))


@torch.library.custom_op("effimvs::encoder_tail_ctx", mutates_args=("hx",))
@_on_tensor_device
def encoder_tail_ctx(m: Tensor, w_m: Tensor, ctx: Tensor, ctx_offset: int, cx: int, ctx_relu: bool, w_ctx: Tensor, bias: Tensor,
                     hx: Tensor) -> None:
    m, ctx = _nhwc(m, "encoder_tail_ctx"), _nhwc(ctx, "encoder_tail_ctx")
    w_m, w_ctx, bias = _dev(w_m, "encoder_tail_ctx"), _dev(w_ctx, "encoder_tail_ctx"), _dev(bias, "encoder_tail_ctx")
    if not (hx.is_cuda and hx.dtype == torch.float32 and hx.is_contiguous(memory_format=torch.channels_last)):
        raise RuntimeError("effimvs::encoder_tail_ctx needs hx as a channels-last fp32 CUDA tensor (it is updated in place)")
    B, hm, H, W = m.shape
    h = w_m.shape[0]
    ct = ctx.shape[1]
    if (hx.shape[1] != 2 * h or w_m.numel() != h * hm or w_ctx.numel() != h * cx or bias.numel() != h or ctx_offset < 0
            or ctx_offset + cx > ct or ctx_offset % 4 or tuple(ctx.shape[2:]) != (H, W)):
        raise ValueError("encoder_tail_ctx: shapes do not match")
    _count(1)
    capi.check(_lib.effimvs_encoder_tail_ctx_f32(m.data_ptr(), w_m.data_ptr(), ctx.data_ptr() + 4 * ctx_offset, ct, cx, int(ctx_relu),
                                                 w_ctx.data_ptr(), bias.data_ptr(), B * H * W, hm, h, hx.data_ptr(), _stream()))


def _conv2d_fns(precision: str):
    if precision == "f16":
        return (_lib.effimvs_conv2d_tf32_supported, _lib.effimvs_conv2d_tf32_packed_bytes, _lib.effimvs_conv2d_tf32_pack,
                _lib.effimvs_conv2d_tf32)
    if precision == "bf16x3":
        return (_lib.effimvs_conv2d_bf16x3_supported, _lib.effimvs_conv2d_bf16x3_packed_bytes, _lib.effimvs_conv2d_bf16x3_pack,
                _lib.effimvs_conv2d_bf16x3)
    raise ValueError("conv2d_tc: precision must be 'f16' or 'bf16x3', got {!r}".format(precision))


def conv2d_tc_supported(cin: int, cout: int, precision: str = "f16") -> bool:
    return bool(_conv2d_fns(precision)[0](int(cin), int(cout)))


def _cl_view(t: Tensor, name: str):
    if not t.is_cuda or t.dtype != torch.float32 or t.dim() != 4:
        raise RuntimeError("effimvs::conv2d_tc needs 4-D fp32 CUDA tensors ({})".format(name))
    B, C, H, W = t.shape
    ps = t.stride(3)
    if t.stride(1) != 1 or t.stride(2) != W * ps or (B > 1 and t.stride(0) != H * W * ps) or ps < C:
        raise RuntimeError("effimvs::conv2d_tc: {} must be a channels-last map or a channel slice of one, got strides {}".format(name, t.stride()))
    return t.data_ptr(), ps


@torch.library.custom_op("effimvs::conv2d_tc_pack", mutates_args=())
@_on_tensor_device
def conv2d_tc_pack(weight: Tensor, precision: str = "f16") -> Tensor:
    supported, packed_bytes, pack, _ = _conv2d_fns(precision)
    weight = _dev(weight, "conv2d_tc_pack")
    cout, cin = weight.shape[:2]
    if tuple(weight.shape[2:]) != (3, 3) or not supported(cin, cout):
        raise ValueError("conv2d_tc_pack: unsupported weight shape {} for precision {}".format(tuple(weight.shape), precision))
    packed = torch.empty(packed_bytes(cin, cout) // 4, device=weight.device, dtype=torch.float32)
    _count(1)
    capi.check(pack(weight.data_ptr(), cin, cout, packed.data_ptr(), _stream()))
    return packed


@conv2d_tc_pack.register_fake
def _(weight, precision="f16"):
    copies = 2 if precision == "bf16x3" else 1
    return weight.new_empty(copies * 9 * weight.shape[1] * ((weight.shape[0] + 15) // 16 * 16) // 2)


@torch.library.custom_op("effimvs::conv2d_tc", mutates_args=("out", "aux1"))
@_on_tensor_device
def conv2d_tc(in0: Tensor, in1: Optional[Tensor], packed: Tensor, bias: Optional[Tensor], cout: int, mode: int, out: Tensor,
              aux0: Optional[Tensor], aux1: Optional[Tensor], precision: str = "f16") -> None:
    _, packed_bytes, _, conv = _conv2d_fns(precision)
    B, c0, H, W = in0.shape
    p0, ps0 = _cl_view(in0, "in0")
    p1, ps1, c1 = None, 0, 0
    if in1 is not None:
        p1, ps1 = _cl_view(in1, "in1")
        c1 = in1.shape[1]
        if tuple(in1.shape) != (B, c1, H, W):
            raise ValueError("conv2d_tc: in1 {} does not match in0 {}".format(tuple(in1.shape), tuple(in0.shape)))
    po, pso = _cl_view(out, "out")
    h = cout // 2 if mode == capi.CONV2D_GRU_GATES else cout
    if tuple(out.shape) != (B, h, H, W):
        raise ValueError("conv2d_tc: out {} should be {}".format(tuple(out.shape), (B, h, H, W)))
    pa0, psa0 = _cl_view(aux0, "aux0") if aux0 is not None else (None, 0)
    pa1, psa1 = _cl_view(aux1, "aux1") if aux1 is not None else (None, 0)
    for a in (aux0, aux1):
        if a is not None and tuple(a.shape) != (B, h, H, W):
            raise ValueError("conv2d_tc: aux map {} should be {}".format(tuple(a.shape), (B, h, H, W)))
    if packed.numel() * 4 != packed_bytes(c0 + c1, cout):
        raise ValueError("conv2d_tc: packed weights do not match cin = {} cout = {} ({})".format(c0 + c1, cout, precision))
    bias = _dev(bias, "conv2d_tc") if bias is not None else None
    _count(1)
    capi.check(conv(p0, ps0, c0, p1, ps1, c1, packed.data_ptr(), _opt(bias), cout, B, H, W, mode,
                    po, pso, pa0, psa0, pa1, psa1, _stream()))


@conv2d_tc.register_fake
def _(in0, in1, packed, bias, cout, mode, out, aux0, aux1, precision="f16"):
    return None


@torch.library.custom_op("effimvs::gru_init", mutates_args=())
@_on_tensor_device
def gru_init(ctx_map: Tensor, h: int) -> Tensor:
    ctx_map = _nhwc(ctx_map, "gru_init")
    B, ct, H, W = ctx_map.shape
    if h <= 0 or h % 4 or ct < h or (ct - h) % 4:
        raise ValueError("gru_init: hidden {} / map channels {} must be multiples of 4".format(h, ct))
    hx = torch.empty(B, 2 * h, H, W, device=ctx_map.device, dtype=torch.float32, memory_format=torch.channels_last)
    _count(1)
    capi.check(_lib.effimvs_gru_init_f32(ctx_map.data_ptr(), B * H * W, h, ct - h, hx.data_ptr(), _stream()))
    return hx


@gru_init.register_fake
def _(ctx_map, h):
    B, _, H, W = ctx_map.shape
    return torch.empty((B, 2 * h, H, W), device=ctx_map.device, dtype=ctx_map.dtype, memory_format=torch.channels_last)


@torch.library.custom_op("effimvs::gru_init_ctx", mutates_args=())
@_on_tensor_device
def gru_init_ctx(ctx_map: Tensor, h: int, w_ctx: Tensor, bias: Tensor) -> Tuple[Tensor, Tensor]:
    ctx_map = _nhwc(ctx_map, "gru_init_ctx")
    B, ct, H, W = ctx_map.shape
    cx = ct - h
    if h <= 0 or h % 4 or h > 128 or cx < 4 or cx % 4 or cx > 64:
        raise ValueError("gru_init_ctx: hidden {} (<= 128) / context {} (4..64) channels must be multiples of 4".format(h, cx))
    w2 = w_ctx.detach().reshape(w_ctx.shape[0], -1).contiguous().float()
    if tuple(w2.shape) != (h, cx) or bias.numel() != h:
        raise ValueError("gru_init_ctx: w_ctx {} / bias {} do not match h={}, cx={}".format(tuple(w_ctx.shape), tuple(bias.shape), h, cx))
    bias = bias.detach().contiguous().float()
    hx = torch.empty(B, 2 * h, H, W, device=ctx_map.device, dtype=torch.float32, memory_format=torch.channels_last)
    term = torch.empty(B, h, H, W, device=ctx_map.device, dtype=torch.float32, memory_format=torch.channels_last)
    _count(1)
    capi.check(_lib.effimvs_gru_init_ctx_f32(ctx_map.data_ptr(), B * H * W, h, cx, w2.data_ptr(), bias.data_ptr(), hx.data_ptr(),
                                             term.data_ptr(), _stream()))
    return hx, term


@gru_init_ctx.register_fake
def _(ctx_map, h, w_ctx, bias):
    B, _, H, W = ctx_map.shape
    mk = lambda c: torch.empty((B, c, H, W), device=ctx_map.device, dtype=ctx_map.dtype, memory_format=torch.channels_last)
    return mk(2 * h), mk(h)


@torch.library.custom_op("effimvs::dtu_filter", mutates_args=())
@_on_tensor_device
def dtu_filter(ref_depth: Tensor, srcs_depth: Tensor, conf: Tensor, mats: Tensor, thr_dist: List[float], thr_diff: List[float],
               first_rung: int, full_count: int, conf_thres: float, conf_keep: float, want_masks: bool) -> Tuple[Tensor, Tensor, Tensor, Tensor, Tensor, Tensor]:
    import ctypes
    ref_depth, srcs_depth, conf, mats = (_dev(ref_depth, "dtu_filter"), _dev(srcs_depth, "dtu_filter"), _dev(conf, "dtu_filter"),
                                         _dev(mats, "dtu_filter"))
    v, h, w = srcs_depth.shape
    K = len(thr_dist)
    dev = ref_depth.device
    final = torch.empty(h, w, device=dev, dtype=torch.uint8)
    geo = torch.empty(h, w, device=dev, dtype=torch.uint8)
    avg = torch.empty(h, w, device=dev, dtype=torch.float32)
    pts = torch.empty(3, h, w, device=dev, dtype=torch.float32)
    masks = torch.empty((v, K, h, w) if want_masks else (0,), device=dev, dtype=torch.uint8)
    rep = torch.empty((v, h, w) if want_masks else (0,), device=dev, dtype=torch.float32)
    td = (ctypes.c_double * K)(*thr_dist)
    tf = (ctypes.c_float * K)(*thr_diff)
    _count(1)
    capi.check(_lib.effimvs_dtu_filter_f32(ref_depth.data_ptr(), srcs_depth.data_ptr(), conf.data_ptr(), mats.data_ptr(), td, tf, K,
                                           first_rung, full_count, conf_thres, conf_keep, v, h, w, final.data_ptr(), geo.data_ptr(),
                                           avg.data_ptr(), pts.data_ptr(), masks.data_ptr() if want_masks else None,
                                           rep.data_ptr() if want_masks else None, _stream()))
    return final, geo, avg, pts, masks, rep


@dtu_filter.register_fake
def _(ref_depth, srcs_depth, conf, mats, thr_dist, thr_diff, first_rung, full_count, conf_thres, conf_keep, want_masks):
    v, h, w = srcs_depth.shape
    K = len(thr_dist)
    u8 = torch.uint8
    return (ref_depth.new_empty(h, w, dtype=u8), ref_depth.new_empty(h, w, dtype=u8), ref_depth.new_empty(h, w),
            ref_depth.new_empty(3, h, w), ref_depth.new_empty((v, K, h, w) if want_masks else (0,), dtype=u8),
            ref_depth.new_empty((v, h, w) if want_masks else (0,)))
```

### include/effimvs.h

```cpp
#ifndef EFFIMVS_H
#define EFFIMVS_H

#include <stddef.h>
#include <stdint.h>

#ifdef __cplusplus
extern "C" {
#endif

#define EFFIMVS_OK 0
#define EFFIMVS_EINVAL (-1)
#define EFFIMVS_EUNSUPPORTED (-2)
#define EFFIMVS_ECUDA (-3)
#define EFFIMVS_EWORKSPACE (-4)

#define EFFIMVS_MAX_SRC_VIEWS 16

#define EFFIMVS_HYP_TENSOR 0
#define EFFIMVS_HYP_PLANES 1
#define EFFIMVS_HYP_LOCAL 2

#define EFFIMVS_FEA_NCHW 0
#define EFFIMVS_FEA_NHWC 1

#define EFFIMVS_RANGE_SCALAR 0
#define EFFIMVS_RANGE_PIXEL 1

#define EFFIMVS_PREC_F32 0
#define EFFIMVS_PREC_BF16 1
#define EFFIMVS_PREC_BF16X3 2

const char* effimvs_last_error(void);
int effimvs_version(void);

int effimvs_relative_projection_f32(const float* cams, int B, int V, float* proj_out, void* stream);

int effimvs_homo_warp_f32(const float* src_fea, const float* proj, const float* hyp, int hyp_mode,
                          int B, int C, int H, int W, int D, float* warped_out, void* stream);

int effimvs_depth_ranges_f32(const float* depth_values, int B, int Dv, int D1, const float* ratios3, float* out, void* stream);

int effimvs_depth_range_samples_f32(const float* cur, const float* interval, int B, int ndepth, int H, int W,
                                    float* samples_out, void* stream);

int effimvs_warp_corr_agg_f32(const float* ref_fea, const float* const* src_fea, int n_src,
                              const float* proj, const float* hyp, int hyp_mode, const float* interval,
                              const float* weights, int B, int C, int H, int W, int D, int G, int fea_layout,
                              float* sim_out, float* hyp_out, void* stream);

int effimvs_warp_corr_views_f32(const float* ref_fea, const float* const* src_fea, int n_src,
                                const float* proj, const float* hyp, int hyp_mode,
                                int B, int C, int H, int W, int D, int fea_layout,
                                float* sims_out, float* entropy_out, void* stream);

int effimvs_weighted_agg_f32(const float* sims, const float* weights, int B, int n_src, int D, int H, int W,
                             float* out, void* stream);

int effimvs_volume_lookup_f32(const float* volume, const float* depth_sample, const float* depth_min,
                              const float* depth_max, int range_mode, int sample_stride,
                              int B, int D, int d, int H, int W, float* out, void* stream);

int effimvs_dynamic_cost_f32(const float* cur_depth, const float* raw_volume, const float* reg_volume,
                             const float* interval, const float* depth_min, const float* depth_max,
                             int range_mode, int ndepth, int B, int D, int H, int W, float* out, void* stream);

int effimvs_softmax_regress_conf_f32(const float* prob_pre, const float* hyp, int hyp_mode,
                                     int B, int D, int H, int W, float* depth_out, float* conf_out, void* stream);

int effimvs_conv3d_f32(const float* x, const float* weight, const float* bias, const float* residual,
                       int B, int Cin, int Cout, int D, int H, int W, int sd, int sh, int sw,
                       int transposed, int relu, float* y, int y_coff, int y_ctot, void* stream);

size_t effimvs_conv3d_bf16_workspace_bytes(int B, int Cin, int Cout, int D, int H, int W, int sd, int transposed,
                                           int precision);
int effimvs_conv3d_bf16(const float* x, const float* weight, const float* bias, const float* residual, int B, int Cin,
                        int Cout, int D, int H, int W, int sd, int transposed, int relu, int precision ,
                        void* workspace, size_t workspace_bytes, float* y, void* stream);

size_t effimvs_costreg_workspace_bytes(int B, int D, int H, int W, int precision);
int effimvs_costreg_fpn3d(const float* x, const float* const* weights, const float* const* biases,
                          int B, int D, int H, int W, int precision, void* workspace, size_t workspace_bytes,
                          float* prob_out, void* stream);

size_t effimvs_cost_up_workspace_bytes(int B, int D, int H, int W, int precision);
int effimvs_cost_up_small(const float* x, const float* prev, const float* const* weights,
                          const float* const* biases, int B, int D, int H, int W, int precision,
                          void* workspace, size_t workspace_bytes, float* out, void* stream);

#define EFFIMVS_WS_PREPARE 1
#define EFFIMVS_WS_RUN 2
int effimvs_costreg_fpn3d_ex(const float* x, const float* const* weights, const float* const* biases,
                             int B, int D, int H, int W, int precision, int phases, void* workspace,
                             size_t workspace_bytes, float* prob_out, void* stream);
int effimvs_cost_up_small_ex(const float* x, const float* prev, const float* const* weights,
                             const float* const* biases, int B, int D, int H, int W, int precision, int phases,
                             void* workspace, size_t workspace_bytes, float* out, void* stream);

int effimvs_images_u8_to_f32(const unsigned char* images, long long n, float* out, void* stream);

int effimvs_fusion_reproject_f32(const float* ref_depth, const float* srcs_depth, const float* ref_cam,
                                 const float* srcs_cam, const float* inv_cams, int n, int v, int h, int w,
                                 float* reproj_xyd, void* stream);

int effimvs_fusion_invert_cameras_f32(const float* ref_cam, const float* srcs_cam, int n, int v, float* inv_out, void* stream);

int effimvs_fusion_masks_f32(const float* ref_depth, const float* reproj_xyd, int n, int v, int h, int w,
                             float dist_base, float rel_diff_base, int thres_view, int relative,
                             uint8_t* masks_out, void* stream);

int effimvs_fusion_filter_f32(const float* ref_depth, const float* srcs_depth, const float* conf,
                              const float* ref_cam, const float* srcs_cam, const float* inv_cams,
                              int n, int v, int h, int w, int hc, int wc,
                              float dist_base, float rel_diff_base, int thres_view, float prob_threshold,
                              int relative, uint8_t* final_mask, float* depth_avg, float* points,
                              uint8_t* masks_out, void* stream);


int effimvs_gru_reset_f32(const float* zr_pre, const float* bias_r, const float* hx, long long n_pix, int h, int cx,
                          float* rhx, void* stream);

int effimvs_gru_update_f32(const float* zr_pre, const float* bias_z, const float* q_pre, const float* bias_q, float* hx,
                           long long n_pix, int h, int cx, float* net_out, void* stream);

int effimvs_inv_init_f32(const float* cur_depth, const float* lo_disp, const float* hi_disp, int B, int HW, float* inv_out,
                         float* depth_out, void* stream);

int effimvs_gru_delta_f32(const float* pre, const float* bias, const float* inv, const float* lo_disp, const float* hi_disp,
                          int B, int HW, float* inv_out, float* depth_out, void* stream);

int effimvs_delta_head_f32(const float* t, const float* weight, const float* bias, const float* inv, const float* lo_disp,
                           const float* hi_disp, int B, int h, int H, int W, float* inv_out, float* depth_out, void* stream);

int effimvs_convex_upsample_f32(const float* mask_pre, const float* mask_bias, float mask_scale, const float* inv,
                                const float* lo_disp, const float* hi_disp, int B, int H, int W, int ratio, float* up_out,
                                float* depth_out, void* stream);

int effimvs_convex_upsample_conv_f32(const float* t, int K, const float* mask_w, const float* mask_bias, float mask_scale,
                                     const float* inv, const float* lo_disp, const float* hi_disp, int B, int H, int W, int ratio,
                                     float* up_out, float* depth_out, void* stream);

int effimvs_encoder_head_f32(const float* cost, const float* inv, const float* wc1, const float* bc1, const float* wd1,
                             const float* bd1, int B, int CD, int h, int H, int W, float* out, void* stream);

int effimvs_encoder_head_hostw_f32(const float* cost, const float* inv, const float* host_tables, int B, int CD, int h, int H, int W,
                                   float* out, void* stream);
int effimvs_encoder_head_pack_host(const float* wc1, const float* bc1, const float* wd1, const float* bd1, int CD, int h,
                                   float* tables_out);
int effimvs_encoder_head_table_floats(int h);

int effimvs_encoder_tail_f32(const float* m, const float* w, const float* ctx_term, long long n_pix, int hm, int h,
                             float* hx, void* stream);

int effimvs_encoder_tail_ctx_f32(const float* m, const float* w_m, const float* ctx, int ctx_stride, int cx, int ctx_relu,
                                 const float* w_ctx, const float* bias, long long n_pix, int hm, int h, float* hx, void* stream);

int effimvs_gru_init_f32(const float* ctx_map, long long n_pix, int h, int cx, float* hx, void* stream);

int effimvs_gru_init_ctx_f32(const float* ctx_map, long long n_pix, int h, int cx, const float* w_ctx, const float* bias,
                             float* hx, float* ctx_term, void* stream);

#define EFFIMVS_CONV2D_BIAS 0
#define EFFIMVS_CONV2D_BIAS_RELU 1
#define EFFIMVS_CONV2D_ADD_RELU 2
#define EFFIMVS_CONV2D_GRU_GATES 3
#define EFFIMVS_CONV2D_GRU_UPDATE 4

int effimvs_conv2d_tf32_supported(int cin, int cout);
size_t effimvs_conv2d_tf32_packed_bytes(int cin, int cout);
int effimvs_conv2d_tf32_pack(const float* w, int cin, int cout, void* packed, void* stream);
int effimvs_conv2d_tf32(const float* in0, long long in0_pixstride, int c0, const float* in1, long long in1_pixstride, int c1,
                        const void* packed, const float* bias, int cout, int B, int H, int W, int mode,
                        float* out, long long out_pixstride, const float* aux0, long long aux0_pixstride,
                        float* aux1, long long aux1_pixstride, void* stream);

int effimvs_conv2d_bf16x3_supported(int cin, int cout);
size_t effimvs_conv2d_bf16x3_packed_bytes(int cin, int cout);
int effimvs_conv2d_bf16x3_pack(const float* w, int cin, int cout, void* packed, void* stream);
int effimvs_conv2d_bf16x3(const float* in0, long long in0_pixstride, int c0, const float* in1, long long in1_pixstride, int c1,
                          const void* packed, const float* bias, int cout, int B, int H, int W, int mode,
                          float* out, long long out_pixstride, const float* aux0, long long aux0_pixstride,
                          float* aux1, long long aux1_pixstride, void* stream);

int effimvs_dtu_filter_f32(const float* ref_depth, const float* srcs_depth, const float* conf, const float* mats,
                           const double* thr_dist_host, const float* thr_diff_host, int n_rungs, int first_rung,
                           int full_count, float conf_thres, float conf_keep, int v, int h, int w,
                           uint8_t* final_mask, uint8_t* geo_mask, float* depth_avg, float* points, uint8_t* masks_out,
                           float* reproj_depth_out, void* stream);

#ifdef __cplusplus
}
#endif
#endif
```

Baseline: 165.6.

## Fuse small-resolution GRU refinement iterations into one persistent row-pipelined kernel

```diff
diff --git a/effi-mvs-plus_b200/capi.py b/effi-mvs-plus_b200/capi.py
--- a/effi-mvs-plus_b200/capi.py
+++ b/effi-mvs-plus_b200/capi.py
@@ -79,6 +79,11 @@
                                  _p, C.c_longlong, _p, C.c_longlong, _p, C.c_longlong, _p]),
     "effimvs_gru_init_f32": (_i, [_p, C.c_longlong, _i, _i, _p, _p]),
     "effimvs_gru_init_ctx_f32": (_i, [_p, C.c_longlong, _i, _i, _p, _p, _p, _p, _p]),
+    "effimvs_gru_small_supported": (_i, [_i, _i, _i]),
+    "effimvs_gru_small_packed_bytes": (_sz, [_i, _i, _i]),
+    "effimvs_gru_small_pack": (_i, [_p] * 19 + [_i, _i, _i, _p, _p]),
+    "effimvs_gru_small_workspace_bytes": (_sz, [_i, _i, _i, _i]),
+    "effimvs_gru_small_f32": (_i, [_p] * 10 + [_i] * 8 + [_p, _p, _p, _p, _p, _sz, _p]),
     "effimvs_dtu_filter_f32": (_i, [_p, _p, _p, _p, C.POINTER(C.c_double), C.POINTER(C.c_float), _i, _i, _i, _f, _f, _i, _i, _i,
                                     _p, _p, _p, _p, _p, _p, _p]),
     "effimvs_images_u8_to_f32": (_i, [_p, C.c_longlong, _p, _p]),
diff --git a/effi-mvs-plus_b200/csrc/gru_small.cu b/effi-mvs-plus_b200/csrc/gru_small.cu
--- /dev/null
+++ b/effi-mvs-plus_b200/csrc/gru_small.cu
@@ -0,0 +1,765 @@
+#include <cuda_fp16.h>
+
+#include "common.cuh"
+
+namespace effimvs {
+namespace {
+
+constexpr int GS_THREADS = 512, GS_WARPS = GS_THREADS / 32;
+constexpr int GS_MAX_W = 256, GS_MAX_H = 48;
+constexpr int GS_PHASES = 7;
+constexpr int HC_MAX_NT = GS_MAX_H / 8;
+constexpr long long GS_SPIN_CAP = 1ll << 22;
+constexpr int GS_CTRL_BYTES = 256;
+
+struct GsLayout {
+    long long cd2[2], dp[2], zr[2], q[2], hd, mk;
+    long long img_halves;
+    long long wc1, bc1, wd1, bd1, bcd2, wctx, bctx, bzr, bq, bh1, wd2, bd2, bm0, f32_floats;
+    __host__ __device__ GsLayout(int h, int cx, int cd) {
+        const long long s = 9ll * (h + 8);
+        long long o = 0;
+        cd2[0] = o; o += s * h; cd2[1] = o; o += s * h;
+        dp[0] = o; o += s * h; dp[1] = o; o += s * h;
+        zr[0] = o; o += s * 2 * h; zr[1] = o; o += s * 2 * h;
+        q[0] = o; o += s * h; q[1] = o; o += s * h;
+        hd = o; o += s * h;
+        mk = o; o += s * 2 * h;
+        img_halves = (o + 7) / 8 * 8;
+        long long f = 0;
+        wc1 = f; f += (long long)h * cd; bc1 = f; f += h; wd1 = f; f += 49ll * h; bd1 = f; f += h; bcd2 = f; f += 2 * h;
+        wctx = f; f += (long long)h * cx; bctx = f; f += h; bzr = f; f += 2 * h; bq = f; f += h; bh1 = f; f += h;
+        wd2 = f; f += 9ll * h; bd2 = f; f += 4; bm0 = f; f += 2 * h;
+        f32_floats = f;
+    }
+    __host__ __device__ size_t bytes() const { return (size_t)img_halves * 2 + (size_t)f32_floats * 4; }
+};
+
+struct GsParams {
+    const float* ctx_map;
+    const float* raw; const float* reg;
+    const float* interval; const float* vmin; const float* vmax;
+    const float* cur_depth;
+    const float* lo; const float* hi;
+    const __half* img; const float* f32;
+    float* net;
+    float* inv_all; float* depth_all;
+    float* m0;
+    int* ctrl;
+    __half *c1d1, *cd, *x, *rh, *t1;
+    __half* h16;
+    float *z, *ctxt;
+    int B, H, W, cx, cost_num, D, iters;
+#ifdef GS_TRACE
+    unsigned long long* trace;
+#endif
+};
+
+__device__ __forceinline__ int ld_acquire(const int* p) {
+    int v;
+    asm volatile("ld.acquire.gpu.global.b32 %0, [%1];" : "=r"(v) : "l"(p) : "memory");
+    return v;
+}
+__device__ __forceinline__ void st_release(int* p, int v) { asm volatile("st.release.gpu.global.b32 [%0], %1;" ::"l"(p), "r"(v) : "memory"); }
+__device__ __forceinline__ float ld_cgf(const float* p) { return __ldcg(p); }
+__device__ __forceinline__ float2 ld_cgf2(const float* p) { return __ldcg(reinterpret_cast<const float2*>(p)); }
+__device__ __forceinline__ void cp_async16(void* smem, const void* gmem, int bytes = 16) {
+    asm volatile("cp.async.cg.shared.global [%0], [%1], 16, %2;" ::"r"((uint32_t)__cvta_generic_to_shared(smem)), "l"(gmem), "r"(bytes)
+                 : "memory");
+}
+__device__ __forceinline__ void cp_async_wait_all() { asm volatile("cp.async.wait_all;" ::: "memory"); }
+__device__ __forceinline__ void cp_async_commit() { asm volatile("cp.async.commit_group;" ::: "memory"); }
+template <int N>
+__device__ __forceinline__ void cp_async_wait() { asm volatile("cp.async.wait_group %0;" ::"n"(N) : "memory"); }
+
+__device__ __forceinline__ float sigmoid_t(float x) { return __fdividef(1.0f, 1.0f + __expf(-x)); }
+__device__ __forceinline__ float tanh_t(float x) { return 1.0f - __fdividef(2.0f, 1.0f + __expf(2.0f * x)); }
+__device__ __forceinline__ float to_depth(float inv, float lo, float hi) {
+    const float s = fmaxf(__fadd_rn(lo, __fmul_rn(__fsub_rn(hi, lo), inv)), 1e-4f);
+    return __fdiv_rn(1.0f, s);
+}
+
+__device__ __forceinline__ float local_hypothesis(float cur_depth, float interval, int D, int d) {
+    float inv = __fdiv_rn(1.0f, cur_depth);
+    float half = __fmul_rn((float)(D / 2), interval);
+    float lo = fmaxf(__fsub_rn(inv, half), 1e-4f);
+    float hi = fminf(fmaxf(__fadd_rn(inv, half), 1e-4f), 1e4f);
+    float step = __fmul_rn(__fsub_rn(hi, lo), __fdiv_rn(1.0f, (float)(D - 1)));
+    float s = fmaxf(__fadd_rn(lo, __fmul_rn((float)d, step)), 1e-5f);
+    return __fdiv_rn(1.0f, s);
+}
+__device__ __forceinline__ float lookup_1d(const float* __restrict__ vol, int D, int HW, float depth, float dmin, float dmax) {
+    float inv_max = __fdiv_rn(1.0f, dmax);
+    float num = __fsub_rn(__fdiv_rn(1.0f, depth), inv_max);
+    float den = __fadd_rn(__fsub_rn(__fdiv_rn(1.0f, dmin), inv_max), 1e-10f);
+    float t = __fmul_rn(__fdiv_rn(num, den), (float)(D - 1));
+    float g = __fsub_rn(__fmul_rn(__fmul_rn(2.0f, t), __fdiv_rn(1.0f, (float)(D - 1))), 1.0f);
+    float ix = __fmul_rn(__fmul_rn(__fadd_rn(g, 1.0f), 0.5f), (float)(D - 1));
+    float f = floorf(ix);
+    float w1 = __fsub_rn(ix, f);
+    float w0 = __fsub_rn(__fadd_rn(f, 1.0f), ix);
+    float out = 0.0f;
+    if (f >= 0.0f && f <= (float)(D - 1)) out = __fmul_rn(__ldg(vol + (size_t)((int)f) * HW), w0);
+    if (f >= -1.0f && f <= (float)(D - 2)) out = fmaf(__ldg(vol + (size_t)((int)f + 1) * HW), w1, out);
+    return out;
+}
+
+template <int HC>
+struct Gs {
+    static constexpr int S = HC + 8;
+    static constexpr int NT = HC / 8;
+    static constexpr int KS = HC / 16;
+    static constexpr int W_HALVES = 9 * 2 * HC * S;
+    static constexpr int IN_HALVES = 3 * (GS_MAX_W + 2) * S;
+    static constexpr size_t SMEM = (size_t)(W_HALVES + IN_HALVES) * 2 + 64;
+};
+
+struct Smem {
+    __half* w;
+    __half* in;
+    int* abort;
+};
+
+__device__ bool wait_rows(const GsParams& P, const Smem& sm, int b, int y, int r, int target) {
+    if (threadIdx.x < 2 * r + 1) {
+        const int yy = y - r + (int)threadIdx.x;
+        if (yy >= 0 && yy < P.H) {
+            const int* f = reinterpret_cast<const int*>(reinterpret_cast<const char*>(P.ctrl) + GS_CTRL_BYTES) + b * P.H + yy;
+            long long n = 0;
+            while (ld_acquire(f) < target) {
+                if (++n > GS_SPIN_CAP || ld_acquire(P.ctrl) != 0) {
+                    atomicExch(P.ctrl, 1);
+                    *sm.abort = 1;
+                    break;
+                }
+                if (n > 32) __nanosleep(n < 1024 ? 64 : 512);
+            }
+        }
+    }
+    __syncthreads();
+#ifdef GS_TRACE
+    if (threadIdx.x == 0) {
+        unsigned long long t;
+        asm volatile("mov.u64 %0, %globaltimer;" : "=l"(t));
+        P.trace[((size_t)(b * P.H + y) * 64 + target + 1) * 2] = t;
+    }
+#endif
+    return *sm.abort == 0;
+}
+
+#ifdef GS_TRACE
+#define GS_MARK(g, slot)                                                                                    \
+    do {                                                                                                    \
+        __syncthreads();                                                                                    \
+        if (threadIdx.x == 0) {                                                                             \
+            unsigned long long t_;                                                                          \
+            asm volatile("mov.u64 %0, %globaltimer;" : "=l"(t_));                                          \
+            P.trace[((size_t)(g) * 64 + (slot)) * 2] = t_;                                                  \
+        }                                                                                                   \
+    } while (0)
+#else
+#define GS_MARK(g, slot) do {} while (0)
+#endif
+
+__device__ __forceinline__ void publish(const GsParams& P, int g, int step) {
+    GS_MARK(g, 24 + step);
+    __syncthreads();
+    if (threadIdx.x == 0) {
+        st_release(reinterpret_cast<int*>(reinterpret_cast<char*>(P.ctrl) + GS_CTRL_BYTES) + g, step);
+#ifdef GS_TRACE
+        unsigned long long t;
+        asm volatile("mov.u64 %0, %globaltimer;" : "=l"(t));
+        P.trace[((size_t)g * 64 + step) * 2 + 1] = t;
+#endif
+    }
+}
+
+template <int HC>
+__device__ __forceinline__ void stage_weights(const Smem& sm, const __half* src, int cout, int tg) {
+    const int per_tap = cout * Gs<HC>::S / 8, i0 = 3 * tg * per_tap, n16 = i0 + 3 * per_tap;
+    for (int i = i0 + (int)threadIdx.x; i < n16; i += GS_THREADS) cp_async16(sm.w + 8 * i, src + 8 * i);
+}
+
+template <int HC, bool F32>
+__device__ void stage_rows(const GsParams& P, const Smem& sm, const void* map, int cs, int coff, int b, int y) {
+    constexpr int S = Gs<HC>::S, V = HC / 8;
+    const int Wp = (P.W + 15) & ~15, SW = Wp + 2, n = 3 * SW * V;
+    if (!F32) {
+        for (int i = threadIdx.x; i < n; i += GS_THREADS) {
+            const int v = i % V, col = (i / V) % SW, r = i / (V * SW);
+            const int yy = y + r - 1, xx = col - 1;
+            const bool in = yy >= 0 && yy < P.H && xx >= 0 && xx < P.W;
+            const long long pix = in ? ((long long)b * P.H + yy) * P.W + xx : 0;
+            cp_async16(sm.in + ((size_t)r * SW + col) * S + 8 * v, reinterpret_cast<const __half*>(map) + pix * cs + coff + 8 * v, in ? 16 : 0);
+        }
+        return;
+    }
+    constexpr int GS_RB = 4;
+    for (int i0 = 0; i0 < n; i0 += GS_THREADS * GS_RB) {
+        float4 a[GS_RB][2];
+#pragma unroll
+        for (int k = 0; k < GS_RB; ++k) {
+            const int i = i0 + k * GS_THREADS + (int)threadIdx.x;
+            const int v = i % V, col = (i / V) % SW, r = i / (V * SW);
+            const int yy = y + r - 1, xx = col - 1;
+            a[k][0] = a[k][1] = make_float4(0.0f, 0.0f, 0.0f, 0.0f);
+            if (i < n && yy >= 0 && yy < P.H && xx >= 0 && xx < P.W) {
+                const float4* s = reinterpret_cast<const float4*>(reinterpret_cast<const float*>(map) + (((long long)b * P.H + yy) * P.W + xx) * cs + coff + 8 * v);
+                a[k][0] = __ldcg(s);
+                a[k][1] = __ldcg(s + 1);
+            }
+        }
+#pragma unroll
+        for (int k = 0; k < GS_RB; ++k) {
+            const int i = i0 + k * GS_THREADS + (int)threadIdx.x;
+            if (i >= n) break;
+            const int v = i % V, col = (i / V) % SW, r = i / (V * SW);
+            __half2 h[4] = {__floats2half2_rn(a[k][0].x, a[k][0].y), __floats2half2_rn(a[k][0].z, a[k][0].w),
+                            __floats2half2_rn(a[k][1].x, a[k][1].y), __floats2half2_rn(a[k][1].z, a[k][1].w)};
+            *reinterpret_cast<uint4*>(sm.in + ((size_t)r * SW + col) * S + 8 * v) = *reinterpret_cast<uint4*>(h);
+        }
+    }
+}
+
+__device__ __forceinline__ void ldsm_x4(uint32_t& r0, uint32_t& r1, uint32_t& r2, uint32_t& r3, const void* p) {
+    asm volatile("ldmatrix.sync.aligned.m8n8.x4.shared.b16 {%0,%1,%2,%3}, [%4];"
+                 : "=r"(r0), "=r"(r1), "=r"(r2), "=r"(r3)
+                 : "r"((uint32_t)__cvta_generic_to_shared(p)));
+}
+__device__ __forceinline__ void mma16816(float* d, uint32_t a0, uint32_t a1, uint32_t a2, uint32_t a3, uint32_t b0, uint32_t b1) {
+    asm volatile("mma.sync.aligned.m16n8k16.row.col.f32.f16.f16.f32 {%0,%1,%2,%3}, {%4,%5,%6,%7}, {%8,%9}, {%0,%1,%2,%3};"
+                 : "+f"(d[0]), "+f"(d[1]), "+f"(d[2]), "+f"(d[3])
+                 : "r"(a0), "r"(a1), "r"(a2), "r"(a3), "r"(b0), "r"(b1));
+}
+
+struct Frag {
+    uint32_t a[4], b[HC_MAX_NT][2];
+};
+template <int HC>
+__device__ __forceinline__ void load_frag(Frag& f, const __half* a_base, const __half* b_base, int k, int SW, int cout) {
+    constexpr int S = Gs<HC>::S, NT = Gs<HC>::NT, KS = Gs<HC>::KS;
+    const int tap = k / KS, ks = k - tap * KS, ky = tap / 3, kx = tap - 3 * ky;
+    ldsm_x4(f.a[0], f.a[1], f.a[2], f.a[3], a_base + (size_t)(ky * SW + kx) * S + 16 * ks);
+    const __half* bp = b_base + (size_t)tap * cout * S + 16 * ks;
+#pragma unroll
+    for (int t = 0; t < NT; t += 2) ldsm_x4(f.b[t][0], f.b[t][1], f.b[t + 1][0], f.b[t + 1][1], bp + (size_t)(8 * t) * S);
+}
+template <int HC>
+__device__ __forceinline__ void mma_frag(float (&acc)[HC / 8][4], const Frag& f) {
+#pragma unroll
+    for (int t = 0; t < HC / 8; ++t) mma16816(acc[t], f.a[0], f.a[1], f.a[2], f.a[3], f.b[t][0], f.b[t][1]);
+}
+
+template <int HC, int TG>
+__device__ __forceinline__ void mma_taps(const Smem& sm, float (&acc)[2][HC / 8][4], int nm, int n_groups_total, int g_lo, int n_groups,
+                                         int SW) {
+    constexpr int S = Gs<HC>::S, KS = Gs<HC>::KS, K0 = 3 * TG * KS, K1 = K0 + 3 * KS;
+    const int warp = threadIdx.x >> 5, lane = threadIdx.x & 31;
+    const int j = lane >> 3, r8 = lane & 7;
+    const int cout = n_groups * HC;
+#pragma unroll
+    for (int it = 0; it < 2; ++it) {
+        const int item = warp + GS_WARPS * it;
+        if (item >= nm * n_groups_total) continue;
+        const int grp = item / nm, mt = item - grp * nm;
+        if (grp < g_lo || grp >= g_lo + n_groups) continue;
+        const __half* a_base = sm.in + (size_t)(mt * 16 + r8 + 8 * (j & 1)) * S + 8 * (j >> 1);
+        const __half* b_base = sm.w + (size_t)((grp - g_lo) * HC + 8 * (j >> 1) + r8) * S + 8 * (j & 1);
+        Frag f0, f1;
+        load_frag<HC>(f0, a_base, b_base, K0, SW, cout);
+#pragma unroll
+        for (int k = K0; k < K1; k += 2) {
+            if (k + 1 < K1) load_frag<HC>(f1, a_base, b_base, k + 1, SW, cout);
+            mma_frag<HC>(acc[it], f0);
+            if (k + 1 < K1) {
+                if (k + 2 < K1) load_frag<HC>(f0, a_base, b_base, k + 2, SW, cout);
+                mma_frag<HC>(acc[it], f1);
+            }
+        }
+    }
+}
+
+struct Chunk {
+    const void* map; int cs, coff; bool f32;
+    const __half* w; int g_lo, n_groups;
+};
+
+template <int HC, int NC, class Aux, class Epi>
+__device__ bool conv_row(const GsParams& P, const Smem& sm, const Chunk (&ch)[NC], int n_groups_total, int b, int y, int wait_step, Aux aux,
+                         Epi epi) {
+    constexpr int NT = Gs<HC>::NT;
+    const int Wp = (P.W + 15) & ~15, nm = Wp / 16;
+    float acc[2][NT][4];
+#pragma unroll
+    for (int i = 0; i < 2; ++i)
+#pragma unroll
+        for (int t = 0; t < NT; ++t) acc[i][t][0] = acc[i][t][1] = acc[i][t][2] = acc[i][t][3] = 0.0f;
+#pragma unroll
+    for (int c = 0; c < NC; ++c) {
+        const int cout = ch[c].n_groups * HC, SW = Wp + 2;
+        stage_weights<HC>(sm, ch[c].w, cout, 0);
+        cp_async_commit();
+        if (c == 0 && wait_step > 0 && !wait_rows(P, sm, b, y, 1, wait_step)) return false;
+        if (ch[c].f32) stage_rows<HC, true>(P, sm, ch[c].map, ch[c].cs, ch[c].coff, b, y);
+        else stage_rows<HC, false>(P, sm, ch[c].map, ch[c].cs, ch[c].coff, b, y);
+        cp_async_commit();
+        stage_weights<HC>(sm, ch[c].w, cout, 1);
+        cp_async_commit();
+        stage_weights<HC>(sm, ch[c].w, cout, 2);
+        cp_async_commit();
+        cp_async_wait<2>();
+        __syncthreads();
+        if (c == 0 && wait_step == 6) GS_MARK(b * P.H + y, 50);
+        mma_taps<HC, 0>(sm, acc, nm, n_groups_total, ch[c].g_lo, ch[c].n_groups, SW);
+        cp_async_wait<1>();
+        __syncthreads();
+        mma_taps<HC, 1>(sm, acc, nm, n_groups_total, ch[c].g_lo, ch[c].n_groups, SW);
+        cp_async_wait<0>();
+        __syncthreads();
+        mma_taps<HC, 2>(sm, acc, nm, n_groups_total, ch[c].g_lo, ch[c].n_groups, SW);
+        __syncthreads();
+    }
+    if (wait_step == 6) GS_MARK(b * P.H + y, 51);
+    const int warp = threadIdx.x >> 5, lane = threadIdx.x & 31;
+#pragma unroll
+    for (int it = 0; it < 2; ++it) {
+        const int item = warp + GS_WARPS * it;
+        if (item >= nm * n_groups_total) continue;
+        const int grp = item / nm, mt = item - grp * nm;
+        float4 ax[NT][2];
+#pragma unroll
+        for (int t = 0; t < NT; ++t)
+#pragma unroll
+            for (int e = 0; e < 2; ++e) {
+                const int x = mt * 16 + (lane >> 2) + 8 * e, c = 8 * t + 2 * (lane & 3);
+                ax[t][e] = x < P.W ? aux(grp, x, c) : make_float4(0.0f, 0.0f, 0.0f, 0.0f);
+            }
+#pragma unroll
+        for (int t = 0; t < NT; ++t)
+#pragma unroll
+            for (int e = 0; e < 2; ++e) {
+                const int x = mt * 16 + (lane >> 2) + 8 * e, c = 8 * t + 2 * (lane & 3);
+                if (x < P.W) epi(grp, x, c, acc[it][t][2 * e], acc[it][t][2 * e + 1], ax[t][e]);
+            }
+    }
+    return true;
+}
+
+template <int HC>
+__global__ void __launch_bounds__(GS_THREADS, 1) gru_small_kernel(const GsParams P) {
+    constexpr int h = HC;
+    extern __shared__ __align__(128) uint8_t gsm[];
+    Smem sm;
+    sm.w = reinterpret_cast<__half*>(gsm);
+    sm.in = sm.w + Gs<HC>::W_HALVES;
+    sm.abort = reinterpret_cast<int*>(sm.in + Gs<HC>::IN_HALVES);
+    float* s_f = reinterpret_cast<float*>(sm.in);
+    if (threadIdx.x == 0) *sm.abort = 0;
+    __syncthreads();
+
+    const int cx = P.cx, CD = 2 * P.cost_num, H = P.H, W = P.W;
+    const long long HW = (long long)H * W, BHW = P.B * HW;
+    const GsLayout L(h, cx, CD);
+    const __half* img = P.img;
+    const float* F = P.f32;
+    const int rows = P.B * H;
+
+    for (int g = blockIdx.x; g < rows; g += gridDim.x) {
+        const int b = g / H;
+        const long long p0 = (long long)g * W;
+        for (int i = threadIdx.x; i < W * h; i += GS_THREADS) {
+            const int x = i / h, o = i - x * h;
+            const float* cm = P.ctx_map + (p0 + x) * (h + cx);
+            const float hv = tanhf(__ldg(cm + o));
+            P.net[(p0 + x) * h + o] = hv;
+            P.h16[(p0 + x) * h + o] = __float2half_rn(hv);
+            float acc = __ldg(F + L.bctx + o);
+            for (int k = 0; k < cx; ++k) acc = fmaf(fmaxf(__ldg(cm + h + k), 0.0f), __ldg(F + L.wctx + o * cx + k), acc);
+            P.ctxt[(p0 + x) * h + o] = acc;
+        }
+        const float l = __ldg(P.lo + b), hh = __ldg(P.hi + b);
+        const float span = __fadd_rn(__fsub_rn(hh, l), 1e-10f);
+        for (int x = threadIdx.x; x < W; x += GS_THREADS) {
+            const float v = __fdiv_rn(__fsub_rn(__frcp_rn(__ldg(P.cur_depth + p0 + x)), l), span);
+            P.inv_all[p0 + x] = v;
+            P.depth_all[p0 + x] = to_depth(v, l, hh);
+        }
+        publish(P, g, 1);
+    }
+
+    for (int iter = 0; iter < P.iters; ++iter) {
+        const float* inv = P.inv_all + iter * BHW;
+        const float* dep = P.depth_all + iter * BHW;
+        const int s0 = 2 + iter * GS_PHASES;
+        for (int g = blockIdx.x; g < rows; g += gridDim.x) {
+            const int b = g / H, y = g - b * H;
+            const long long p0 = (long long)g * W;
+            float* s_cost = s_f;
+            float* s_inv = s_f + GS_MAX_W * 8;
+            const int IW = W + 7;
+            float* s_wd = reinterpret_cast<float*>(sm.w);
+            float* s_wc = s_wd + 49 * h;
+            float* s_b = s_wc + 8 * h;
+            for (int i = threadIdx.x; i < 49 * h; i += GS_THREADS) s_wd[i] = __ldg(F + L.wd1 + (i % h) * 49 + i / h);
+            for (int i = threadIdx.x; i < CD * h; i += GS_THREADS) s_wc[i] = __ldg(F + L.wc1 + (i % h) * CD + i / h);
+            for (int i = threadIdx.x; i < 2 * h; i += GS_THREADS) s_b[i] = __ldg(F + (i < h ? L.bc1 + i : L.bd1 + i - h));
+            for (int x = threadIdx.x; x < W; x += GS_THREADS) {
+                const float cur = ld_cgf(dep + p0 + x), iv = __ldg(P.interval + b);
+                const float dmin = __ldg(P.vmin + b), dmax = __ldg(P.vmax + b);
+                const float* vraw = P.raw + (size_t)b * P.D * HW + (long long)y * W + x;
+                const float* vreg = P.reg + (size_t)b * P.D * HW + (long long)y * W + x;
+                for (int k = 0; k < P.cost_num; ++k) {
+                    const float d = local_hypothesis(cur, iv, P.cost_num, k);
+                    s_cost[x * 8 + k] = lookup_1d(vraw, P.D, (int)HW, d, dmin, dmax);
+                    s_cost[x * 8 + P.cost_num + k] = lookup_1d(vreg, P.D, (int)HW, d, dmin, dmax);
+                }
+            }
+            if (!wait_rows(P, sm, b, y, 3, s0 - 1)) return;
+            for (int i = threadIdx.x; i < 7 * IW; i += GS_THREADS) {
+                const int r = i / IW, xx = i - r * IW - 3, yy = y + r - 3;
+                s_inv[i] = (yy >= 0 && yy < H && xx >= 0 && xx < W) ? ld_cgf(inv + ((long long)b * H + yy) * W + xx) : 0.0f;
+            }
+            __syncthreads();
+            constexpr int CH = h / 2;
+            for (int i = threadIdx.x; i < 4 * ((W + 1) / 2); i += GS_THREADS) {
+                const int q = i / ((W + 1) / 2), x = 2 * (i - q * ((W + 1) / 2));
+                const bool two = x + 1 < W;
+                const int o0 = (q & 1) * CH;
+                float acc[2][CH];
+                if (q < 2) {
+#pragma unroll
+                    for (int j = 0; j < CH; ++j) acc[0][j] = acc[1][j] = s_b[o0 + j];
+                    for (int c = 0; c < CD; ++c) {
+                        const float v0 = s_cost[x * 8 + c], v1 = s_cost[(two ? x + 1 : x) * 8 + c];
+                        const float4* wp = reinterpret_cast<const float4*>(s_wc + c * h + o0);
+#pragma unroll
+                        for (int k = 0; k < CH / 4; ++k) {
+                            const float4 wv = wp[k];
+                            acc[0][4 * k] = fmaf(v0, wv.x, acc[0][4 * k]); acc[0][4 * k + 1] = fmaf(v0, wv.y, acc[0][4 * k + 1]);
+                            acc[0][4 * k + 2] = fmaf(v0, wv.z, acc[0][4 * k + 2]); acc[0][4 * k + 3] = fmaf(v0, wv.w, acc[0][4 * k + 3]);
+                            acc[1][4 * k] = fmaf(v1, wv.x, acc[1][4 * k]); acc[1][4 * k + 1] = fmaf(v1, wv.y, acc[1][4 * k + 1]);
+                            acc[1][4 * k + 2] = fmaf(v1, wv.z, acc[1][4 * k + 2]); acc[1][4 * k + 3] = fmaf(v1, wv.w, acc[1][4 * k + 3]);
+                        }
+                    }
+                } else {
+#pragma unroll
+                    for (int j = 0; j < CH; ++j) acc[0][j] = acc[1][j] = s_b[h + o0 + j];
+                    for (int ty = 0; ty < 7; ++ty) {
+                        float v[8];
+#pragma unroll
+                        for (int k = 0; k < 8; ++k) v[k] = s_inv[ty * IW + x + k];
+#pragma unroll
+                        for (int tx = 0; tx < 7; ++tx) {
+                            const float4* wp = reinterpret_cast<const float4*>(s_wd + (ty * 7 + tx) * h + o0);
+#pragma unroll
+                            for (int k = 0; k < CH / 4; ++k) {
+                                const float4 wv = wp[k];
+                                acc[0][4 * k] = fmaf(v[tx], wv.x, acc[0][4 * k]); acc[0][4 * k + 1] = fmaf(v[tx], wv.y, acc[0][4 * k + 1]);
+                                acc[0][4 * k + 2] = fmaf(v[tx], wv.z, acc[0][4 * k + 2]); acc[0][4 * k + 3] = fmaf(v[tx], wv.w, acc[0][4 * k + 3]);
+                                acc[1][4 * k] = fmaf(v[tx + 1], wv.x, acc[1][4 * k]); acc[1][4 * k + 1] = fmaf(v[tx + 1], wv.y, acc[1][4 * k + 1]);
+                                acc[1][4 * k + 2] = fmaf(v[tx + 1], wv.z, acc[1][4 * k + 2]);
+                                acc[1][4 * k + 3] = fmaf(v[tx + 1], wv.w, acc[1][4 * k + 3]);
+                            }
+                        }
+                    }
+                }
+#pragma unroll
+                for (int p = 0; p < 2; ++p) {
+                    if (p == 1 && !two) break;
+                    uint4* dst = reinterpret_cast<uint4*>(P.c1d1 + (p0 + x + p) * (2 * h) + q * CH);
+#pragma unroll
+                    for (int k = 0; k < CH / 8; ++k) {
+                        __half2 o[4];
+#pragma unroll
+                        for (int j = 0; j < 4; ++j)
+                            o[j] = __floats2half2_rn(fmaxf(acc[p][8 * k + 2 * j], 0.0f), fmaxf(acc[p][8 * k + 2 * j + 1], 0.0f));
+                        dst[k] = *reinterpret_cast<uint4*>(o);
+                    }
+                }
+            }
+            publish(P, g, s0);
+        }
+        for (int g = blockIdx.x; g < rows; g += gridDim.x) {
+            const int b = g / H, y = g - b * H;
+            const long long p0 = (long long)g * W;
+            const Chunk ch[2] = {{P.c1d1, 2 * h, 0, false, img + L.cd2[0], 0, 1}, {P.c1d1, 2 * h, h, false, img + L.cd2[1], 1, 1}};
+            const bool ok = conv_row<HC>(P, sm, ch, 2, b, y, s0, [](int, int, int) { return make_float4(0.0f, 0.0f, 0.0f, 0.0f); }, [&](int grp, int x, int c, float v0, float v1, float4) {
+                const int o = grp * h + c;
+                *reinterpret_cast<__half2*>(P.cd + (p0 + x) * (2 * h) + o) =
+                    __floats2half2_rn(fmaxf(__fadd_rn(v0, __ldg(F + L.bcd2 + o)), 0.0f), fmaxf(__fadd_rn(v1, __ldg(F + L.bcd2 + o + 1)), 0.0f));
+            });
+            if (!ok) return;
+            publish(P, g, s0 + 1);
+        }
+        for (int g = blockIdx.x; g < rows; g += gridDim.x) {
+            const int b = g / H, y = g - b * H;
+            const long long p0 = (long long)g * W;
+            const Chunk ch[2] = {{P.cd, 2 * h, 0, false, img + L.dp[0], 0, 1}, {P.cd, 2 * h, h, false, img + L.dp[1], 0, 1}};
+            const bool ok = conv_row<HC>(P, sm, ch, 1, b, y, s0 + 1,
+                [&](int, int x, int c) { const float2 t = ld_cgf2(P.ctxt + (p0 + x) * h + c); return make_float4(t.x, t.y, 0.0f, 0.0f); },
+                [&](int, int x, int c, float v0, float v1, float4 a) {
+                    *reinterpret_cast<__half2*>(P.x + (p0 + x) * h + c) =
+                        __floats2half2_rn(fmaxf(__fadd_rn(v0, a.x), 0.0f), fmaxf(__fadd_rn(v1, a.y), 0.0f));
+                });
+            if (!ok) return;
+            publish(P, g, s0 + 2);
+        }
+        for (int g = blockIdx.x; g < rows; g += gridDim.x) {
+            const int b = g / H, y = g - b * H;
+            const long long p0 = (long long)g * W;
+            const Chunk ch[2] = {{P.h16, h, 0, false, img + L.zr[0], 0, 2}, {P.x, h, 0, false, img + L.zr[1], 0, 2}};
+            const bool ok = conv_row<HC>(P, sm, ch, 2, b, y, s0 + 2,
+                [&](int grp, int x, int c) {
+                    const float2 t = grp ? ld_cgf2(P.net + (p0 + x) * h + c) : make_float2(0.0f, 0.0f);
+                    return make_float4(t.x, t.y, 0.0f, 0.0f);
+                },
+                [&](int grp, int x, int c, float v0, float v1, float4 a) {
+                    const long long o = (p0 + x) * h + c;
+                    const float s0 = sigmoid_t(__fadd_rn(v0, __ldg(F + L.bzr + grp * h + c)));
+                    const float s1 = sigmoid_t(__fadd_rn(v1, __ldg(F + L.bzr + grp * h + c + 1)));
+                    if (grp == 0) *reinterpret_cast<float2*>(P.z + o) = make_float2(s0, s1);
+                    else *reinterpret_cast<__half2*>(P.rh + o) = __floats2half2_rn(__fmul_rn(s0, a.x), __fmul_rn(s1, a.y));
+                });
+            if (!ok) return;
+            publish(P, g, s0 + 3);
+        }
+        for (int g = blockIdx.x; g < rows; g += gridDim.x) {
+            const int b = g / H, y = g - b * H;
+            const long long p0 = (long long)g * W;
+            const Chunk ch[2] = {{P.rh, h, 0, false, img + L.q[0], 0, 1}, {P.x, h, 0, false, img + L.q[1], 0, 1}};
+            const bool ok = conv_row<HC>(P, sm, ch, 1, b, y, s0 + 3,
+                [&](int, int x, int c) {
+                    const float2 z = ld_cgf2(P.z + (p0 + x) * h + c), hv = ld_cgf2(P.net + (p0 + x) * h + c);
+                    return make_float4(z.x, z.y, hv.x, hv.y);
+                },
+                [&](int, int x, int c, float v0, float v1, float4 a) {
+                    const float q0 = tanh_t(__fadd_rn(v0, __ldg(F + L.bq + c))), q1 = tanh_t(__fadd_rn(v1, __ldg(F + L.bq + c + 1)));
+                    const float h0 = __fadd_rn(__fmul_rn(__fsub_rn(1.0f, a.x), a.z), __fmul_rn(a.x, q0));
+                    const float h1 = __fadd_rn(__fmul_rn(__fsub_rn(1.0f, a.y), a.w), __fmul_rn(a.y, q1));
+                    *reinterpret_cast<float2*>(P.net + (p0 + x) * h + c) = make_float2(h0, h1);
+                    *reinterpret_cast<__half2*>(P.h16 + (p0 + x) * h + c) = __floats2half2_rn(h0, h1);
+                });
+            if (!ok) return;
+            publish(P, g, s0 + 4);
+        }
+        for (int g = blockIdx.x; g < rows; g += gridDim.x) {
+            const int b = g / H, y = g - b * H;
+            const long long p0 = (long long)g * W;
+            const Chunk ch[1] = {{P.h16, h, 0, false, img + L.hd, 0, 1}};
+            const bool ok = conv_row<HC>(P, sm, ch, 1, b, y, s0 + 4, [](int, int, int) { return make_float4(0.0f, 0.0f, 0.0f, 0.0f); }, [&](int, int x, int c, float v0, float v1, float4) {
+                *reinterpret_cast<__half2*>(P.t1 + (p0 + x) * h + c) =
+                    __floats2half2_rn(fmaxf(__fadd_rn(v0, __ldg(F + L.bh1 + c)), 0.0f), fmaxf(__fadd_rn(v1, __ldg(F + L.bh1 + c + 1)), 0.0f));
+            });
+            if (!ok) return;
+            publish(P, g, s0 + 5);
+        }
+        for (int g = blockIdx.x; g < rows; g += gridDim.x) {
+            const int b = g / H, y = g - b * H;
+            const long long p0 = (long long)g * W;
+            constexpr int S = Gs<HC>::S;
+            const int SW = ((W + 15) & ~15) + 2;
+            float* s_w2 = reinterpret_cast<float*>(sm.w);
+            for (int i = threadIdx.x; i < 9 * h; i += GS_THREADS) s_w2[i] = __ldg(F + L.wd2 + (i % h) * 9 + i / h);
+            if (!wait_rows(P, sm, b, y, 1, s0 + 5)) return;
+            stage_rows<HC, false>(P, sm, P.t1, h, 0, b, y);
+            cp_async_wait_all();
+            __syncthreads();
+            if (iter == 0) GS_MARK(g, 48);
+            for (int i0 = 0; i0 < 4 * W; i0 += GS_THREADS) {
+                const int i = i0 + (int)threadIdx.x, x = i >> 2, q = i & 3;
+                float acc = 0.0f;
+                if (x < W) {
+#pragma unroll
+                    for (int tap = 0; tap < 9; ++tap) {
+                        const int ky = tap / 3, kx = tap - 3 * ky;
+                        const __half2* sp = reinterpret_cast<const __half2*>(sm.in + ((size_t)ky * SW + x + kx) * S + q * (h / 4));
+                        const float2* wp = reinterpret_cast<const float2*>(s_w2 + tap * h + q * (h / 4));
+#pragma unroll
+                        for (int c2 = 0; c2 < h / 8; ++c2) {
+                            const float2 v = __half22float2(sp[c2]), wv = wp[c2];
+                            acc = fmaf(v.x, wv.x, acc);
+                            acc = fmaf(v.y, wv.y, acc);
+                        }
+                    }
+                }
+                acc += __shfl_xor_sync(0xffffffffu, acc, 1);
+                acc += __shfl_xor_sync(0xffffffffu, acc, 2);
+                if (q == 0 && x < W) {
+                    const float v = __fadd_rn(ld_cgf(inv + p0 + x), tanhf(__fadd_rn(acc, __ldg(F + L.bd2))));
+                    P.inv_all[(iter + 1) * BHW + p0 + x] = v;
+                    P.depth_all[(iter + 1) * BHW + p0 + x] = to_depth(v, __ldg(P.lo + b), __ldg(P.hi + b));
+                }
+            }
+            if (iter == 0) GS_MARK(g, 49);
+            publish(P, g, s0 + 6);
+        }
+    }
+    for (int g = blockIdx.x; g < rows; g += gridDim.x) {
+        const int b = g / H, y = g - b * H;
+        const long long p0 = (long long)g * W;
+        const Chunk ch[1] = {{P.h16, h, 0, false, img + L.mk, 0, 2}};
+        const int last = P.iters > 0 ? 2 + P.iters * GS_PHASES - 1 : 1;
+        const bool ok = conv_row<HC>(P, sm, ch, 2, b, y, last, [](int, int, int) { return make_float4(0.0f, 0.0f, 0.0f, 0.0f); }, [&](int grp, int x, int c, float v0, float v1, float4) {
+            const int o = grp * h + c;
+            *reinterpret_cast<float2*>(P.m0 + (p0 + x) * (2 * h) + o) =
+                make_float2(fmaxf(__fadd_rn(v0, __ldg(F + L.bm0 + o)), 0.0f), fmaxf(__fadd_rn(v1, __ldg(F + L.bm0 + o + 1)), 0.0f));
+        });
+        if (!ok) return;
+    }
+}
+
+__global__ void gs_pack_conv_kernel(const float* __restrict__ w, int cin_total, int ci0, int co0, int cn, int h, __half* __restrict__ out) {
+    const int S = h + 8;
+    const int n = 9 * cn * S;
+    for (int i = blockIdx.x * blockDim.x + threadIdx.x; i < n; i += gridDim.x * blockDim.x) {
+        const int k = i % S, o = (i / S) % cn, tap = i / (S * cn);
+        out[i] = k < h ? __float2half_rn(w[((size_t)(co0 + o) * cin_total + ci0 + k) * 9 + tap]) : __float2half_rn(0.0f);
+    }
+}
+
+__global__ void gs_copy_kernel(const float* __restrict__ src, int n, float* __restrict__ dst) {
+    for (int i = blockIdx.x * blockDim.x + threadIdx.x; i < n; i += gridDim.x * blockDim.x) dst[i] = src[i];
+}
+
+}
+}
+
+using namespace effimvs;
+
+extern "C" int effimvs_gru_small_supported(int h, int cx, int W) {
+    return (h == 16 || h == 32 || h == 48) && (cx == 4 || cx == 8 || cx == 12) && W >= 1 && W <= GS_MAX_W;
+}
+
+extern "C" size_t effimvs_gru_small_packed_bytes(int h, int cx, int cost_num) {
+    if (!effimvs_gru_small_supported(h, cx, 1) || cost_num < 1 || cost_num > 4) return 0;
+    return GsLayout(h, cx, 2 * cost_num).bytes();
+}
+
+extern "C" int effimvs_gru_small_pack(const float* w_cd2, const float* b_cd2, const float* w_dprime, const float* w_zr, const float* b_zr,
+                                      const float* w_q, const float* b_q, const float* w_head1, const float* b_head1, const float* w_d2,
+                                      const float* b_d2, const float* w_mask0, const float* b_mask0, const float* w_c1, const float* b_c1,
+                                      const float* w_d1, const float* b_d1, const float* w_ctx, const float* b_ctx, int h, int cx,
+                                      int cost_num, void* out, void* stream) {
+    EFFI_REQUIRE(w_cd2 && b_cd2 && w_dprime && w_zr && b_zr && w_q && b_q && w_head1 && b_head1 && w_d2 && b_d2 && w_mask0 && b_mask0 &&
+                     w_c1 && b_c1 && w_d1 && b_d1 && w_ctx && b_ctx && out,
+                 EFFIMVS_EINVAL, "gru_small_pack: null pointer");
+    EFFI_REQUIRE(effimvs_gru_small_packed_bytes(h, cx, cost_num) > 0, EFFIMVS_EUNSUPPORTED,
+                 "gru_small_pack: h=%d (16/32/48), cx=%d (4/8/12), cost_num=%d (1..4) not supported", h, cx, cost_num);
+    EFFI_REQUIRE((reinterpret_cast<uintptr_t>(out) & 15) == 0, EFFIMVS_EINVAL, "gru_small_pack: out must be 16-byte aligned");
+    cudaStream_t st = (cudaStream_t)stream;
+    const GsLayout L(h, cx, 2 * cost_num);
+    __half* img = reinterpret_cast<__half*>(out);
+    float* f = reinterpret_cast<float*>(img + L.img_halves);
+    auto conv = [&](const float* w, int cin_total, int ci0, int co0, int cn, long long off) {
+        gs_pack_conv_kernel<<<64, 256, 0, st>>>(w, cin_total, ci0, co0, cn, h, img + off);
+    };
+    conv(w_cd2, 2 * h, 0, 0, h, L.cd2[0]);
+    conv(w_cd2, 2 * h, h, h, h, L.cd2[1]);
+    conv(w_dprime, 2 * h, 0, 0, h, L.dp[0]);
+    conv(w_dprime, 2 * h, h, 0, h, L.dp[1]);
+    conv(w_zr, 2 * h, 0, 0, 2 * h, L.zr[0]);
+    conv(w_zr, 2 * h, h, 0, 2 * h, L.zr[1]);
+    conv(w_q, 2 * h, 0, 0, h, L.q[0]);
+    conv(w_q, 2 * h, h, 0, h, L.q[1]);
+    conv(w_head1, h, 0, 0, h, L.hd);
+    conv(w_mask0, h, 0, 0, 2 * h, L.mk);
+    auto copy = [&](const float* src, int n, long long off) { gs_copy_kernel<<<8, 256, 0, st>>>(src, n, f + off); };
+    const int CD = 2 * cost_num;
+    copy(w_c1, h * CD, L.wc1); copy(b_c1, h, L.bc1); copy(w_d1, 49 * h, L.wd1); copy(b_d1, h, L.bd1); copy(b_cd2, 2 * h, L.bcd2);
+    copy(w_ctx, h * cx, L.wctx); copy(b_ctx, h, L.bctx); copy(b_zr, 2 * h, L.bzr); copy(b_q, h, L.bq); copy(b_head1, h, L.bh1);
+    copy(w_d2, 9 * h, L.wd2); copy(b_d2, 1, L.bd2); copy(b_mask0, 2 * h, L.bm0);
+    return check_launch("gs_pack_kernels");
+}
+
+namespace {
+struct GsWs {
+    size_t c1d1, cd, x, rh, t1, h16, z, ctxt, total;
+    GsWs(int B, int H, int W, int h) {
+        const size_t P = (size_t)B * H * W;
+        auto al = [](size_t v) { return (v + 255) / 256 * 256; };
+        size_t o = al(GS_CTRL_BYTES + (size_t)B * H * sizeof(int));
+        c1d1 = o; o += al(P * 2 * h * 2);
+        cd = o; o += al(P * 2 * h * 2);
+        x = o; o += al(P * h * 2);
+        rh = o; o += al(P * h * 2);
+        t1 = o; o += al(P * h * 2);
+        h16 = o; o += al(P * h * 2);
+        z = o; o += al(P * h * 4);
+        ctxt = o; o += al(P * h * 4);
+#ifdef GS_TRACE
+        o += (size_t)B * H * 64 * 2 * 8;
+#endif
+        total = o;
+    }
+};
+}
+
+extern "C" size_t effimvs_gru_small_workspace_bytes(int B, int H, int W, int h) {
+    if (B <= 0 || H <= 0 || W <= 0 || h <= 0) return 0;
+    return GsWs(B, H, W, h).total;
+}
+
+extern "C" int effimvs_gru_small_f32(const float* ctx_map, const float* raw, const float* reg, const float* interval, const float* vmin,
+                                     const float* vmax, const float* cur_depth, const float* lo_disp, const float* hi_disp, const void* packed,
+                                     int B, int H, int W, int h, int cx, int cost_num, int D, int iters, float* net, float* inv_all,
+                                     float* depth_all, float* m0, void* workspace, size_t workspace_bytes, void* stream) {
+    EFFI_REQUIRE(ctx_map && raw && reg && interval && vmin && vmax && cur_depth && lo_disp && hi_disp && packed && net && inv_all && depth_all &&
+                     m0 && workspace,
+                 EFFIMVS_EINVAL, "gru_small: null pointer");
+    EFFI_REQUIRE(B > 0 && H > 0 && D > 1 && iters >= 0 && iters <= 64, EFFIMVS_EINVAL, "gru_small: bad sizes");
+    EFFI_REQUIRE(effimvs_gru_small_supported(h, cx, W) && cost_num >= 1 && cost_num <= 4, EFFIMVS_EUNSUPPORTED,
+                 "gru_small: h=%d (16/32/48), cx=%d (4/8/12), W=%d (<= %d), cost_num=%d (1..4) not supported", h, cx, W, GS_MAX_W, cost_num);
+    const GsWs ws(B, H, W, h);
+    EFFI_REQUIRE(workspace_bytes >= ws.total, EFFIMVS_EWORKSPACE, "gru_small: workspace of %zu bytes, %zu needed", workspace_bytes, ws.total);
+    EFFI_REQUIRE(((reinterpret_cast<uintptr_t>(ctx_map) | reinterpret_cast<uintptr_t>(net) | reinterpret_cast<uintptr_t>(packed) |
+                   reinterpret_cast<uintptr_t>(workspace)) & 15) == 0,
+                 EFFIMVS_EINVAL, "gru_small: maps, packed weights and workspace must be 16-byte aligned");
+    int dev = 0, sms = 0, coop = 0;
+    cudaGetDevice(&dev);
+    cudaDeviceGetAttribute(&sms, cudaDevAttrMultiProcessorCount, dev);
+    cudaDeviceGetAttribute(&coop, cudaDevAttrCooperativeLaunch, dev);
+    EFFI_REQUIRE(coop, EFFIMVS_EUNSUPPORTED, "gru_small: the device cannot launch cooperative kernels");
+    cudaStream_t st = (cudaStream_t)stream;
+    uint8_t* w8 = reinterpret_cast<uint8_t*>(workspace);
+    if (cudaMemsetAsync(w8, 0, GS_CTRL_BYTES + (size_t)B * H * sizeof(int), st) != cudaSuccess) return check_launch("gru_small: counter reset");
+
+    GsParams P;
+    P.ctx_map = ctx_map; P.raw = raw; P.reg = reg; P.interval = interval; P.vmin = vmin; P.vmax = vmax; P.cur_depth = cur_depth;
+    P.lo = lo_disp; P.hi = hi_disp;
+    const GsLayout L(h, cx, 2 * cost_num);
+    P.img = reinterpret_cast<const __half*>(packed);
+    P.f32 = reinterpret_cast<const float*>(P.img + L.img_halves);
+    P.net = net; P.inv_all = inv_all; P.depth_all = depth_all; P.m0 = m0;
+    P.ctrl = reinterpret_cast<int*>(w8);
+    P.c1d1 = reinterpret_cast<__half*>(w8 + ws.c1d1); P.cd = reinterpret_cast<__half*>(w8 + ws.cd);
+    P.x = reinterpret_cast<__half*>(w8 + ws.x); P.rh = reinterpret_cast<__half*>(w8 + ws.rh); P.t1 = reinterpret_cast<__half*>(w8 + ws.t1);
+    P.h16 = reinterpret_cast<__half*>(w8 + ws.h16);
+    P.z = reinterpret_cast<float*>(w8 + ws.z); P.ctxt = reinterpret_cast<float*>(w8 + ws.ctxt);
+#ifdef GS_TRACE
+    P.trace = reinterpret_cast<unsigned long long*>(w8 + ws.total - (size_t)B * H * 64 * 2 * 8);
+#endif
+    P.B = B; P.H = H; P.W = W; P.cx = cx; P.cost_num = cost_num; P.D = D; P.iters = iters;
+
+    void (*kern)(const GsParams) = nullptr;
+    size_t smem = 0;
+    switch (h) {
+        case 16: kern = gru_small_kernel<16>; smem = Gs<16>::SMEM; break;
+        case 32: kern = gru_small_kernel<32>; smem = Gs<32>::SMEM; break;
+        default: kern = gru_small_kernel<48>; smem = Gs<48>::SMEM; break;
+    }
+    if (cudaFuncSetAttribute(kern, cudaFuncAttributeMaxDynamicSharedMemorySize, (int)smem) != cudaSuccess)
+        return check_launch("gru_small: shared memory attribute");
+    const int rows = B * H;
+    cudaLaunchConfig_t cfg = {};
+    cfg.gridDim = dim3(rows < sms ? rows : sms);
+    cfg.blockDim = dim3(GS_THREADS);
+    cfg.dynamicSmemBytes = smem;
+    cfg.stream = st;
+    cudaLaunchAttribute attr[1];
+    attr[0].id = cudaLaunchAttributeCooperative;
+    attr[0].val.cooperative = 1;
+    cfg.attrs = attr;
+    cfg.numAttrs = 1;
+    cudaLaunchKernelEx(&cfg, kern, P);
+    return check_launch("gru_small_kernel");
+}
diff --git a/effi-mvs-plus_b200/hotpath.py b/effi-mvs-plus_b200/hotpath.py
--- a/effi-mvs-plus_b200/hotpath.py
+++ b/effi-mvs-plus_b200/hotpath.py
@@ -255,6 +255,14 @@
     conv2d_tc = staticmethod(ops.conv2d_tc)
     conv2d_tc_pack = staticmethod(ops.conv2d_tc_pack)
     conv2d_tc_supported = staticmethod(ops.conv2d_tc_supported)
+    gru_small_supported = staticmethod(ops.gru_small_supported)
+    gru_small_pack = staticmethod(ops.gru_small_pack)
+
+    def gru_small(self, ctx_map, raw, reg, interval, vmin, vmax, cur_depth, lo_disp, hi_disp, packed, h, cost_num, iters):
+        B = raw.shape[0]
+        iv = interval.reshape(-1).expand(B) if torch.is_tensor(interval) else torch.full((B,), float(interval), device=raw.device)
+        return ops.gru_small(ctx_map, raw, reg, iv.float().contiguous(), vmin.reshape(B), vmax.reshape(B), cur_depth, lo_disp.reshape(B),
+                             hi_disp.reshape(B), packed, h, cost_num, iters)
 
     def softmax_regress_conf(self, prob_pre, hyp):
         if _is_planes(hyp):
diff --git a/effi-mvs-plus_b200/net.py b/effi-mvs-plus_b200/net.py
--- a/effi-mvs-plus_b200/net.py
+++ b/effi-mvs-plus_b200/net.py
@@ -241,8 +241,10 @@
             inv_seq.append(inv_depth)
         return net, 0.25 * self.mask[2](_conv_relu_mod(self.mask[0], net)), inv_seq
 
-    def forward_fused(self, glue, net, cost_fn, inv_depth, context, iters, lo_disp, hi_disp, ctx_map=None, want_mask=True, cur_depth=None):
-        return update_block_forward_fused(self, glue, net, cost_fn, inv_depth, context, iters, lo_disp, hi_disp, ctx_map, want_mask, cur_depth)
+    def forward_fused(self, glue, net, cost_fn, inv_depth, context, iters, lo_disp, hi_disp, ctx_map=None, want_mask=True, cur_depth=None,
+                      cost_args=None):
+        return update_block_forward_fused(self, glue, net, cost_fn, inv_depth, context, iters, lo_disp, hi_disp, ctx_map, want_mask, cur_depth,
+                                          cost_args)
 
 
 def _fused_update_weights(block):
@@ -282,14 +284,67 @@
     return env == "1" or H * W >= int(os.environ.get("EFFIMVS_CONV2D_MIN_PIXELS", "100000"))
 
 
+def _gru_small_enabled(glue, block, ctx_map, cur_depth, cost_args):
+    if cost_args is None or ctx_map is None or cur_depth is None or not hasattr(glue, "gru_small"):
+        return False
+    if os.environ.get("EFFIMVS_CONV2D", "auto") in ("0", "1") or getattr(glue, "conv2d_fp32_grade", False):
+        return False
+    if not torch.backends.cudnn.allow_tf32:
+        return False
+    g, e, hd = block.depth_gru, block.encoder, block.depth_head
+    h = g.convz.out_channels
+    cx = e.convc.in_channels - e.convd.out_channels
+    raw, _, _, near, far, cost_num = cost_args
+    B, _, H, W = ctx_map.shape
+    if (ctx_map.shape[1] != h + cx or e.convc1.in_channels != 2 * cost_num or tuple(hd.conv2.weight.shape) != (1, h, 3, 3)
+            or tuple(block.mask[2].kernel_size) != (1, 1) or block.mask[2].out_channels != 36
+            or raw.shape[0] != B or tuple(raw.shape[2:]) != (H, W) or near.numel() != B or far.numel() != B):
+        return False
+    if not glue.gru_small_supported(h, cx, W):
+        return False
+    return H * W < int(os.environ.get("EFFIMVS_CONV2D_MIN_PIXELS", "100000"))
+
+
+def _d_prime(e):
+    hm = e.convd.out_channels
+    return torch.einsum("om,miyx->oiyx", e.convc.weight.detach()[:, :hm, 0, 0], e.convd.weight.detach()).contiguous()
+
+
+def _gru_small_weights(block, glue, w, cost_num):
+    g, e, hd = block.depth_gru, block.encoder, block.depth_head
+    h = g.convz.out_channels
+    cx = e.convc.in_channels - e.convd.out_channels
+    key = ("gru_small", cost_num)
+    packed = w.get(key)
+    if packed is None:
+        d = lambda t: t.detach().contiguous()
+        packed = glue.gru_small_pack([
+            d(w["w_cd2"]), d(w["b_cd2"]), _d_prime(e), d(w["wzr"]), torch.cat([g.convz.bias.detach(), g.convr.bias.detach()]),
+            d(g.convq.weight), d(g.convq.bias), d(hd.conv1.weight), d(hd.conv1.bias), d(w["w_d2"]), d(hd.conv2.bias),
+            d(block.mask[0].weight), d(block.mask[0].bias), d(e.convc1.weight), d(e.convc1.bias), d(e.convd1.weight), d(e.convd1.bias),
+            d(w["wc_ctx"]), d(w["bias_c"])], h, cx, cost_num)
+        w[key] = packed
+    return packed
+
+
+def _update_block_forward_small(block, glue, w, ctx_map, cost_args, iters, lo_disp, hi_disp, want_mask, cur_depth):
+    raw, reg, interval, near, far, cost_num = cost_args
+    h = block.depth_gru.convz.out_channels
+    ratio = int(round((block.mask[2].out_channels / 9) ** 0.5))
+    packed = _gru_small_weights(block, glue, w, cost_num)
+    net, inv_all, depth_all, m0, _ = glue.gru_small(ctx_map, raw, reg, interval, near, far, cur_depth, lo_disp, hi_disp, packed, h,
+                                                    cost_num, iters)
+    mask_pre = F.conv2d(m0, block.mask[2].weight, None)
+    up, depth_up = glue.convex_upsample(mask_pre, block.mask[2].bias, 0.25, inv_all[iters], lo_disp, hi_disp, ratio)
+    return net, list(inv_all[1:]), list(depth_all[1:]), up, depth_up, (mask_pre if want_mask else None)
+
+
 def _tc_update_weights(block, glue, w):
     key = ("tc", getattr(glue, "conv2d_precision", "f16"))
     tc = w.get(key)
     if tc is None:
         g, e, hd = block.depth_gru, block.encoder, block.depth_head
-        hm = e.convd.out_channels
-        d_prime = torch.einsum("om,miyx->oiyx", e.convc.weight.detach()[:, :hm, 0, 0], e.convd.weight.detach())
-        tc = {"cd2": glue.conv2d_tc_pack(w["w_cd2"]), "dprime": glue.conv2d_tc_pack(d_prime.contiguous()),
+        tc = {"cd2": glue.conv2d_tc_pack(w["w_cd2"]), "dprime": glue.conv2d_tc_pack(_d_prime(e)),
               "zr": glue.conv2d_tc_pack(w["wzr"]), "q": glue.conv2d_tc_pack(g.convq.weight.detach()),
               "head1": glue.conv2d_tc_pack(hd.conv1.weight.detach()), "mask0": glue.conv2d_tc_pack(block.mask[0].weight.detach()),
               "b_zr": torch.cat([g.convz.bias.detach(), g.convr.bias.detach()]).contiguous()}
@@ -340,8 +395,10 @@
 
 
 def update_block_forward_fused(block, glue, net, cost_fn, inv_depth, context, iters, lo_disp, hi_disp, ctx_map=None, want_mask=True,
-                               cur_depth=None):
+                               cur_depth=None, cost_args=None):
     w = _fused_update_weights(block)
+    if _gru_small_enabled(glue, block, ctx_map, cur_depth, cost_args):
+        return _update_block_forward_small(block, glue, w, ctx_map, cost_args, iters, lo_disp, hi_disp, want_mask, cur_depth)
     g, e, hd = block.depth_gru, block.encoder, block.depth_head
     ratio = int(round((block.mask[2].out_channels / 9) ** 0.5))
     h = g.convz.out_channels
@@ -544,7 +601,8 @@
 
             if glue is not None:
                 _, _, depth_seq, _, depth_up, _ = self.update_block[s].forward_fused(
-                    glue, None, cost_fn, None, None, self.iters[s], lo_disp.reshape(B), hi_disp.reshape(B), ctx_pyr[s], False, cur_depth)
+                    glue, None, cost_fn, None, None, self.iters[s], lo_disp.reshape(B), hi_disp.reshape(B), ctx_pyr[s], False, cur_depth,
+                    (raw_vol, reg_vol, interval, vol_near, vol_far, self.cost_num))
                 preds.extend(d.squeeze(1) for d in depth_seq)
                 preds.append(depth_up)
                 continue
diff --git a/effi-mvs-plus_b200/ops.py b/effi-mvs-plus_b200/ops.py
--- a/effi-mvs-plus_b200/ops.py
+++ b/effi-mvs-plus_b200/ops.py
@@ -953,6 +953,74 @@
     return mk(2 * h), mk(h)
 
 
+def gru_small_supported(h: int, cx: int, W: int) -> bool:
+    return bool(_lib.effimvs_gru_small_supported(int(h), int(cx), int(W)))
+
+
+@torch.library.custom_op("effimvs::gru_small_pack", mutates_args=())
+@_on_tensor_device
+def gru_small_pack(weights: List[Tensor], h: int, cx: int, cost_num: int) -> Tensor:
+    nbytes = _lib.effimvs_gru_small_packed_bytes(h, cx, cost_num)
+    if nbytes == 0 or len(weights) != 19:
+        raise ValueError("gru_small_pack: h={}, cx={}, cost_num={} ({} tensors) not supported".format(h, cx, cost_num, len(weights)))
+    ws = [_dev(w.detach(), "gru_small_pack") for w in weights]
+    expect = [4 * h * h * 9, 2 * h, 2 * h * h * 9, 4 * h * h * 9, 2 * h, 2 * h * h * 9, h, h * h * 9, h, h * 9, 1, 2 * h * h * 9, 2 * h,
+              h * 2 * cost_num, h, h * 49, h, h * cx, h]
+    if [w.numel() for w in ws] != expect:
+        raise ValueError("gru_small_pack: tensor sizes {} should be {}".format([w.numel() for w in ws], expect))
+    packed = torch.empty((nbytes + 3) // 4, device=ws[0].device, dtype=torch.float32)
+    _count(23)
+    capi.check(_lib.effimvs_gru_small_pack(*[w.data_ptr() for w in ws], h, cx, cost_num, packed.data_ptr(), _stream()))
+    return packed
+
+
+@gru_small_pack.register_fake
+def _(weights, h, cx, cost_num):
+    return weights[0].new_empty((_lib.effimvs_gru_small_packed_bytes(h, cx, cost_num) + 3) // 4)
+
+
+@torch.library.custom_op("effimvs::gru_small", mutates_args=())
+@_on_tensor_device
+def gru_small(ctx_map: Tensor, raw: Tensor, reg: Tensor, interval: Tensor, vmin: Tensor, vmax: Tensor, cur_depth: Tensor,
+              lo_disp: Tensor, hi_disp: Tensor, packed: Tensor, h: int, cost_num: int, iters: int
+              ) -> Tuple[Tensor, Tensor, Tensor, Tensor, Tensor]:
+    ctx_map = _nhwc(ctx_map, "gru_small")
+    raw, reg, cur_depth = _dev(raw, "gru_small"), _dev(reg, "gru_small"), _dev(cur_depth, "gru_small")
+    interval, vmin, vmax = _dev(interval, "gru_small"), _dev(vmin, "gru_small"), _dev(vmax, "gru_small")
+    lo_disp, hi_disp = _dev(lo_disp, "gru_small"), _dev(hi_disp, "gru_small")
+    B, ct, H, W = ctx_map.shape
+    cx = ct - h
+    D = raw.shape[1]
+    if (tuple(raw.shape) != (B, D, H, W) or reg.shape != raw.shape or cur_depth.numel() != B * H * W or
+            any(t.numel() != B for t in (interval, vmin, vmax, lo_disp, hi_disp))):
+        raise ValueError("gru_small: inconsistent shapes")
+    if not gru_small_supported(h, cx, W):
+        raise ValueError("gru_small: h={}, cx={}, W={} not supported".format(h, cx, W))
+    if packed.numel() != (_lib.effimvs_gru_small_packed_bytes(h, cx, cost_num) + 3) // 4:
+        raise ValueError("gru_small: packed weights do not match h={}, cx={}, cost_num={}".format(h, cx, cost_num))
+    dev = ctx_map.device
+    net = torch.empty(B, h, H, W, device=dev, dtype=torch.float32, memory_format=torch.channels_last)
+    m0 = torch.empty(B, 2 * h, H, W, device=dev, dtype=torch.float32, memory_format=torch.channels_last)
+    inv_all = torch.empty(iters + 1, B, 1, H, W, device=dev, dtype=torch.float32)
+    depth_all = torch.empty(iters + 1, B, 1, H, W, device=dev, dtype=torch.float32)
+    nws = _lib.effimvs_gru_small_workspace_bytes(B, H, W, h)
+    ws = torch.empty(nws, device=dev, dtype=torch.uint8)
+    _count(2)
+    capi.check(_lib.effimvs_gru_small_f32(ctx_map.data_ptr(), raw.data_ptr(), reg.data_ptr(), interval.data_ptr(), vmin.data_ptr(),
+                                          vmax.data_ptr(), cur_depth.data_ptr(), lo_disp.data_ptr(), hi_disp.data_ptr(), packed.data_ptr(),
+                                          B, H, W, h, cx, cost_num, D, iters, net.data_ptr(), inv_all.data_ptr(), depth_all.data_ptr(),
+                                          m0.data_ptr(), ws.data_ptr(), nws, _stream()))
+    return net, inv_all, depth_all, m0, ws
+
+
+@gru_small.register_fake
+def _(ctx_map, raw, reg, interval, vmin, vmax, cur_depth, lo_disp, hi_disp, packed, h, cost_num, iters):
+    B, _, H, W = ctx_map.shape
+    cl = lambda c: torch.empty((B, c, H, W), device=ctx_map.device, dtype=torch.float32, memory_format=torch.channels_last)
+    seq = lambda: ctx_map.new_empty(iters + 1, B, 1, H, W)
+    return cl(h), seq(), seq(), cl(2 * h), ctx_map.new_empty(_lib.effimvs_gru_small_workspace_bytes(B, H, W, h), dtype=torch.uint8)
+
+
 @torch.library.custom_op("effimvs::dtu_filter", mutates_args=())
 @_on_tensor_device
 def dtu_filter(ref_depth: Tensor, srcs_depth: Tensor, conf: Tensor, mats: Tensor, thr_dist: List[float], thr_diff: List[float],
diff --git a/include/effimvs.h b/include/effimvs.h
--- a/include/effimvs.h
+++ b/include/effimvs.h
@@ -181,6 +181,19 @@
                           float* out, long long out_pixstride, const float* aux0, long long aux0_pixstride,
                           float* aux1, long long aux1_pixstride, void* stream);
 
+int effimvs_gru_small_supported(int h, int cx, int W);
+size_t effimvs_gru_small_packed_bytes(int h, int cx, int cost_num);
+int effimvs_gru_small_pack(const float* w_cd2, const float* b_cd2, const float* w_dprime, const float* w_zr, const float* b_zr,
+                           const float* w_q, const float* b_q, const float* w_head1, const float* b_head1, const float* w_d2,
+                           const float* b_d2, const float* w_mask0, const float* b_mask0, const float* w_c1, const float* b_c1,
+                           const float* w_d1, const float* b_d1, const float* w_ctx, const float* b_ctx, int h, int cx, int cost_num,
+                           void* out, void* stream);
+size_t effimvs_gru_small_workspace_bytes(int B, int H, int W, int h);
+int effimvs_gru_small_f32(const float* ctx_map, const float* raw, const float* reg, const float* interval, const float* vmin,
+                          const float* vmax, const float* cur_depth, const float* lo_disp, const float* hi_disp, const void* packed,
+                          int B, int H, int W, int h, int cx, int cost_num, int D, int iters, float* net, float* inv_all,
+                          float* depth_all, float* m0, void* workspace, size_t workspace_bytes, void* stream);
+
 int effimvs_dtu_filter_f32(const float* ref_depth, const float* srcs_depth, const float* conf, const float* mats,
                            const double* thr_dist_host, const float* thr_diff_host, int n_rungs, int first_rung,
                            int full_count, float conf_thres, float conf_keep, int v, int h, int w,
```

Result: no change. 165.2 (median of 6 runs) (-0.2%).
